# marcelodallaqua/TensorDiffEq

Measured on AMD Instinct MI355X. Metric: collocation-pts/sec + L2 rel-error, Allen-Cahn SA-PINN @ 1/2/4/8 GPU, higher is better.
Workload: dtype bf16; 1 GPU; model=Allen-Cahn SA-PINN tanh MLP [2,128,128,128,128,1], problem=ac-sa, global_batch=50000, parallelism=dp1, points_per_gpu=50000, backend=hip, bc_points=IC 512 (SA) + periodic 2x201 (u, u_x)

## Files before the change

tensordiffeq_amd/csrc/jet_bf3.hip:

```cpp
#include "jet_fused3.h"
#include "optim_common.h"

__device__ __forceinline__ void pack_frag(const float* __restrict__ P, bf16x8* __restrict__ img, const NetDims& d,
                                          int WT, int transposed, int e) {
  const int KB = WT / 2;
  {
    const int lane = e & 63, frag = e >> 6;
    const int kb = frag % KB, o = (frag / KB) % WT, layer = frag / (KB * WT) + 1;
    const int p = lane & 15, g = lane >> 4, row = 16 * o + p;
    const float* K = P + off_layer(d, layer);
    bf16x8 hi, lo;
#pragma unroll
    for (int j = 0; j < 8; ++j) {
      const int kf = 32 * kb + (j < 4 ? 4 * g + j : 16 + 4 * g + j - 4);
      const int in = transposed ? kf : row, out = transposed ? row : kf;
      const int win = hw(d, layer - 1), wout = hw(d, layer);
      const float v = (in < win && out < wout) ? K[in * wout + out] : 0.f;
      const __bf16 h = (__bf16)v;
      hi[j] = h;
      lo[j] = (__bf16)(v - (float)h);
    }
    img[(size_t)(frag * 2) * 64 + lane] = hi;
    img[(size_t)(frag * 2 + 1) * 64 + lane] = lo;
  }
}

__device__ __forceinline__ void pack_aux(const float* __restrict__ P, float* __restrict__ aux, const NetDims& d,
                                         int W, int e) {
  {
    float v = 0.f;
    const int w0 = hw(d, 0), wl = hw(d, d.n_hidden - 1);
    if (e < aux_b0(d, W)) {
      const int j = e / W, f = e - j * W;
      if (f < w0) v = P[j * w0 + f];
    } else if (e < aux_bh(d, W)) {
      const int f = e - aux_b0(d, W);
      if (f < w0) v = P[d.d_in * w0 + f];
    } else if (e < aux_ko(d, W)) {
      const int r = e - aux_bh(d, W), i = r / W + 1, f = r - (i - 1) * W;
      if (f < hw(d, i)) v = P[off_layer(d, i) + hw(d, i - 1) * hw(d, i) + f];
    } else if (e < aux_bo(d, W)) {
      const int r = e - aux_ko(d, W), f = r >> 2, q = r & 3;
      if (f < wl && q < d.d_out) v = P[off_layer(d, d.n_hidden) + f * d.d_out + q];
    } else {
      const int q = e - aux_bo(d, W);
      if (q < d.d_out) v = P[off_layer(d, d.n_hidden) + wl * d.d_out + q];
    }
    aux[e] = v;
  }
}

__global__ void __launch_bounds__(256) pack_all_kernel(const float* __restrict__ P, bf16x8* __restrict__ fimg,
                                                       bf16x8* __restrict__ bimg, float* __restrict__ aux, NetDims d,
                                                       int WT) {
  const int nf = (d.n_hidden - 1) * WT * (WT / 2) * 64;
  const int total = 2 * nf + aux_floats(d, 16 * WT);
  for (int e = blockIdx.x * 256 + threadIdx.x; e < total; e += gridDim.x * 256) {
    if (e < nf)
      pack_frag(P, fimg, d, WT, 1, e);
    else if (e < 2 * nf)
      pack_frag(P, bimg, d, WT, 0, e - nf);
    else
      pack_aux(P, aux, d, 16 * WT, e - 2 * nf);
  }
}

struct TailBook {
  const float* lpart;
  int n_lblocks, n_terms, n_scal;
  float* losses;
  float* total;
  float* dscal;
  float* hist;
  int64_t hist_rows;
  int64_t* epoch;
  float* best_loss;
  int64_t* best_epoch;
  int* improved;
  Counters cnt;
};

__global__ void __launch_bounds__(256) tail_reduce1_kernel(const float* __restrict__ slab, float* __restrict__ part,
                                                           int nwg, int Pst, int chunks, int nqb, int half, int c0,
                                                           TailBook tb) {
  if ((int)blockIdx.x < nqb) {
    const int q = blockIdx.x * 256 + threadIdx.x, c = c0 + (int)blockIdx.y;
    if (half) {
      if (8 * q < Pst) slab_reduce1_body8(slab, part, nwg, Pst, chunks, q, c);
    } else if (4 * q < Pst) {
      slab_reduce1_body<false>(slab, part, nwg, Pst, chunks, q, c);
    }
    return;
  }
  if (blockIdx.y != 0) return;
  __shared__ float sh[256];
  const int ns = tb.n_terms + tb.n_scal;
  for (int slot = 0; slot < ns; ++slot) {
    float s = 0.f;
    for (int b = threadIdx.x; b < tb.n_lblocks; b += 256) s += tb.lpart[(size_t)b * ns + slot];
    sh[threadIdx.x] = s;
    __syncthreads();
    for (int k = 128; k > 0; k >>= 1) {
      if ((int)threadIdx.x < k) sh[threadIdx.x] += sh[threadIdx.x + k];
      __syncthreads();
    }
    if (threadIdx.x == 0) {
      if (slot < tb.n_terms) tb.losses[slot] = sh[0];
      else tb.dscal[slot - tb.n_terms] = sh[0];
    }
    __syncthreads();
  }
  if (threadIdx.x == 0 && tb.hist == nullptr && tb.total != nullptr) {
    float s = 0.f;
    for (int t = 0; t < tb.n_terms; ++t) s += tb.losses[t];
    *tb.total = s;
  }
  if (threadIdx.x == 0 && tb.hist != nullptr)
    step_book_body(tb.total, tb.losses, tb.n_terms, 1, tb.hist, tb.hist_rows, tb.epoch, tb.best_loss, tb.best_epoch,
                   tb.improved, tb.cnt);
}

__global__ void __launch_bounds__(256) slab_reduce2_bf3(const float* __restrict__ part, float* __restrict__ grad, int P,
                                                        int Pst, int chunks, const float* __restrict__ gx) {
  const int q = blockIdx.x * 256 + threadIdx.x;
  if (4 * q >= P) return;
  const f32x4 a = slab_reduce2_sum(part, Pst, chunks, q);
#pragma unroll
  for (int e = 0; e < 4; ++e)
    if (4 * q + e < P) grad[4 * q + e] = gx != nullptr ? a[e] + gx[4 * q + e] : a[e];
}

__global__ void __launch_bounds__(256) tail_adam_kernel(AdamArgs args, const float* __restrict__ part, int Pst,
                                                        int chunks, const int* __restrict__ improved,
                                                        float* __restrict__ snap, TailImg ti,
                                                        const float* __restrict__ gx) {
  const bool do_snap = snap != nullptr && *improved != 0;
  const int64_t total = args.start[args.ngroups];
  for (int64_t idx = (int64_t)blockIdx.x * 256 + threadIdx.x; idx < total; idx += (int64_t)gridDim.x * 256) {
    const int gi = adam_group_of(args, idx);
    const AdamGroup gr = args.grp[gi];
    const int64_t e = idx - args.start[gi];
    const bool th = gi == 0;
    float g;
    if (th && part != nullptr) {
      float a0 = 0.f, a1 = 0.f;
      int c = 0;
      for (; c + 7 < chunks; c += 8) {
        float v[8];
#pragma unroll
        for (int k = 0; k < 8; ++k) v[k] = part[(size_t)(c + k) * Pst + e];
#pragma unroll
        for (int k = 0; k < 8; k += 2) {
          a0 += v[k];
          a1 += v[k + 1];
        }
      }
      for (; c + 1 < chunks; c += 2) {
        a0 += part[(size_t)c * Pst + e];
        a1 += part[(size_t)(c + 1) * Pst + e];
      }
      if (c < chunks) a0 += part[(size_t)c * Pst + e];
      g = a0 + a1;
      if (gx != nullptr) g += gx[e];
      const_cast<float*>(gr.g)[e] = g;
    } else {
      g = gr.g[e];
    }
    float p = gr.p[e], m = gr.m[e], v = gr.v[e];
    if (do_snap && th) snap[e] = p;
    adam_elem(p, gr.sign * g, m, v, gr.b1, gr.b2, gr.eps, adam_lr_t(gr));
    gr.p[e] = p;
    gr.m[e] = m;
    gr.v[e] = v;
    if (th && ti.fimg != nullptr) scatter_param(p, (int)e, ti);
  }
}

namespace {

int64_t img_floats(int WT, int n_hidden) {
  return (int64_t)(n_hidden > 1 ? n_hidden - 1 : 0) * WT * (WT / 2) * 128 * 4;
}

int64_t aux_alloc(int d_in, int n_hidden, int W) { return ((int64_t)(d_in + n_hidden + 4) * W + 4 + 3) / 4 * 4; }

int64_t stage_floats(int N, int WT, int S, int lo) {
  const int64_t nwg = (N + 63) / 64;
  return bf3_gstage(WT, S, lo != 0) ? nwg * 4 * stage_wave_elems(WT, S, true) * 2 : 0;
}

int bf3_rows(int N, const NetDims& d, int WT, int S, int lo) {
  const int pts_b = 16 * bwd_waves(WT, lo != 0, S);
  return (N + pts_b - 1) / pts_b;
}

int launch_pack(const float* P, bf16x8* fimg, bf16x8* bimg, float* aux, NetDims d, int WT, hipStream_t st) {
  const int total = 2 * (d.n_hidden - 1) * WT * (WT / 2) * 64 + aux_floats(d, 16 * WT);
  int blocks = (total + 255) / 256;
  if (blocks > 1024) blocks = 1024;
  hipLaunchKernelGGL(pack_all_kernel, dim3(blocks), dim3(256), 0, st, P, fimg, bimg, aux, d, WT);
  TDQ_CHECK_LAUNCH();
  return 0;
}

bool bf3_ok(int WT, int S, int d_in, int d_out, int n_hidden) {
  return (WT == 2 || WT == 4 || WT == 8 || (WT == 16 && S <= 4)) && S >= 1 && S <= TDQ_MAXS &&
         d_in <= TDQ_MAXD && d_out <= TDQ_MAXO && n_hidden >= 1;
}

int dispatch(bool fwd, int WT, int S, int nso, const Bf3Args& a) {
  switch (WT) {
    case 2: return fwd ? bf3_fwd_w2(S, nso, a) : bf3_bwd_w2(S, nso, a);
    case 4: return fwd ? bf3_fwd_w4(S, nso, a) : bf3_bwd_w4(S, nso, a);
    case 8: return fwd ? bf3_fwd_w8(S, nso, a) : bf3_bwd_w8(S, nso, a);
    case 16: return fwd ? bf3_fwd_w16(S, nso, a) : bf3_bwd_w16(S, nso, a);
    default: return (int)hipErrorInvalidValue;
  }
}

}

extern "C" {

int64_t tdq_jet_bf3_scratch_floats(int N, int d_in, const int* widths, int n_hidden, int S, int lo) {
  NetDims d;
  if (!make_dims(d, d_in, widths, 0, 1, n_hidden)) return -1;
  const int WT = width_tiles(d.width);
  if (WT < 2) return -1;
  const int64_t nwg = (N + 63) / 64;
  const int64_t hs = (int64_t)n_hidden * nwg * S * 4 * WT * 256;
  return hs + 2 * img_floats(WT, n_hidden) + aux_alloc(d_in, n_hidden, 16 * WT) + stage_floats(N, WT, S, lo);
}

int64_t tdq_jet_bf3_slab_floats(int N, int d_in, const int* widths, int d_out, int n_hidden) {
  NetDims d;
  if (!make_dims(d, d_in, widths, 0, d_out, n_hidden)) return -1;
  const int WT = width_tiles(d.width);
  if (WT < 2) return -1;
  int nwg = (N + 63) / 64;
  const int fz = (N + 15) / 16 < fz_cus() ? (N + 15) / 16 : fz_cus();
  if (fz > nwg) nwg = fz;
  const int64_t P = slab_stride(param_count(d));
  return ((int64_t)nwg + slab_chunks(nwg)) * P;
}

int64_t tdq_slab_floats_rows(int rows, int d_in, const int* widths, int d_out, int n_hidden) {
  NetDims d;
  if (rows < 1 || !make_dims(d, d_in, widths, 0, d_out, n_hidden)) return -1;
  return ((int64_t)rows + slab_chunks(rows)) * slab_stride(param_count(d));
}

static inline void scratch_images(float* scratch, int n_hidden, int WT, float** img, float** bimg, float** aux) {
  *img = scratch;
  *bimg = *img + img_floats(WT, n_hidden);
  *aux = *bimg + img_floats(WT, n_hidden);
}

static inline bf16x4* scratch_stage(float* scratch, int N, int d_in, int n_hidden, int S, int WT, int lo) {
  if (!bf3_gstage(WT, S, lo != 0)) return nullptr;
  float *img, *bimg, *aux;
  scratch_images(scratch, n_hidden, WT, &img, &bimg, &aux);
  return reinterpret_cast<bf16x4*>(aux + aux_alloc(d_in, n_hidden, 16 * WT));
}

static inline float* scratch_hs(float* scratch, int N, int d_in, int n_hidden, int S, int WT, int lo) {
  return scratch + 2 * img_floats(WT, n_hidden) + aux_alloc(d_in, n_hidden, 16 * WT) + stage_floats(N, WT, S, lo);
}

int tdq_jet_fwd_bf3_range(const float* X, const float* P, float* J, float* scratch, int N, int p_lo, int p_hi,
                          int d_in, const int* widths, int d_out, int n_hidden, int S, const int* spec, int lo, int pack,
                          void* stream) {
  if (N <= 0) return 0;
  if (p_lo < 0 || p_lo % 128 != 0 || p_hi > N || p_hi <= p_lo || (p_hi != N && p_hi % 128 != 0))
    return (int)hipErrorInvalidValue;
  NetDims d;
  if (!make_dims(d, d_in, widths, 0, d_out, n_hidden)) return (int)hipErrorInvalidValue;
  const int WT = width_tiles(d.width);
  JetSpec sp;
  if (!bf3_ok(WT, S, d_in, d_out, n_hidden)) return (int)hipErrorInvalidValue;
  const int nso = spec_nso(S, spec);
  if (nso < 0 || !make_spec(S, spec, sp)) return (int)hipErrorInvalidValue;
  hipStream_t st = reinterpret_cast<hipStream_t>(stream);
  float* Hs = scratch_hs(scratch, N, d_in, n_hidden, S, WT, lo);
  float *img, *bimg, *aux;
  scratch_images(scratch, n_hidden, WT, &img, &bimg, &aux);
  if (pack) {
    int rc = launch_pack(P, reinterpret_cast<bf16x8*>(img), reinterpret_cast<bf16x8*>(bimg), aux, d, WT, st);
    if (rc) return rc;
  }
  Bf3Args a{X, aux, reinterpret_cast<const bf16x8*>(img), nullptr, J, Hs, nullptr, N, 0, d, sp, st, lo,
            scratch_stage(scratch, N, d_in, n_hidden, S, WT, lo), p_lo, p_hi};
  return dispatch(true, WT, S, nso, a);
}

int tdq_jet_fwd_bf3_ex(const float* X, const float* P, float* J, float* scratch, int N, int d_in, const int* widths,
                       int d_out, int n_hidden, int S, const int* spec, int lo, int pack, void* stream) {
  return tdq_jet_fwd_bf3_range(X, P, J, scratch, N, 0, N, d_in, widths, d_out, n_hidden, S, spec, lo, pack, stream);
}

int tdq_jet_fwd_bf3(const float* X, const float* P, float* J, float* scratch, int N, int d_in, const int* widths,
                    int d_out, int n_hidden, int S, const int* spec, int lo, void* stream) {
  return tdq_jet_fwd_bf3_ex(X, P, J, scratch, N, d_in, widths, d_out, n_hidden, S, spec, lo, 1, stream);
}

int tdq_jet_bf3_pack(const float* P, float* scratch, int N, int d_in, const int* widths, int d_out, int n_hidden, int S,
                     void* stream) {
  NetDims d;
  if (!make_dims(d, d_in, widths, 0, d_out, n_hidden)) return (int)hipErrorInvalidValue;
  const int WT = width_tiles(d.width);
  if (!bf3_ok(WT, S, d_in, d_out, n_hidden)) return (int)hipErrorInvalidValue;
  float *img, *bimg, *aux;
  scratch_images(scratch, n_hidden, WT, &img, &bimg, &aux);
  return launch_pack(P, reinterpret_cast<bf16x8*>(img), reinterpret_cast<bf16x8*>(bimg), aux, d, WT,
                     reinterpret_cast<hipStream_t>(stream));
}

int tdq_jet_bwd_bf3_range(const float* X, const float* dJ, const float* Hs, float* work, int N, int p_lo, int p_hi,
                          int d_in, const int* widths, int d_out, int n_hidden, int S, const int* spec, int lo,
                          void* stream) {
  if (N <= 0) return 0;
  if (p_lo < 0 || p_lo % 128 != 0 || p_hi > N || p_hi <= p_lo || (p_hi != N && p_hi % 128 != 0))
    return (int)hipErrorInvalidValue;
  NetDims d;
  if (!make_dims(d, d_in, widths, 0, d_out, n_hidden)) return (int)hipErrorInvalidValue;
  const int WT = width_tiles(d.width);
  JetSpec sp;
  if (!bf3_ok(WT, S, d_in, d_out, n_hidden)) return (int)hipErrorInvalidValue;
  const int nso = spec_nso(S, spec);
  if (nso < 0 || !make_spec(S, spec, sp)) return (int)hipErrorInvalidValue;
  hipStream_t st = reinterpret_cast<hipStream_t>(stream);
  const int Ptot = param_count(d);
  float* scr = const_cast<float*>(Hs);
  float *img, *bimg, *aux;
  scratch_images(scr, n_hidden, WT, &img, &bimg, &aux);
  Bf3Args a{X, aux, reinterpret_cast<const bf16x8*>(bimg), dJ, nullptr, scratch_hs(scr, N, d_in, n_hidden, S, WT, lo),
            work, N, slab_stride(Ptot), d, sp, st, lo, scratch_stage(scr, N, d_in, n_hidden, S, WT, lo), p_lo, p_hi};
  return dispatch(false, WT, S, nso, a);
}

int tdq_jet_bwd_bf3_ex(const float* X, const float* P, const float* dJ, const float* Hs, float* work, float* grad,
                       int N, int d_in, const int* widths, int d_out, int n_hidden, int S, const int* spec, int lo, int reduce,
                       void* stream) {
  if (N <= 0) return 0;
  (void)P;
  int rc = tdq_jet_bwd_bf3_range(X, dJ, Hs, work, N, 0, N, d_in, widths, d_out, n_hidden, S, spec, lo, stream);
  if (rc || !reduce) return rc;
  NetDims d;
  make_dims(d, d_in, widths, 0, d_out, n_hidden);
  const int WT = width_tiles(d.width);
  const int nwg_b = bf3_rows(N, d, WT, S, lo);
  const int Ptot = param_count(d);
  return tdq_slab_reduce_h(work, grad, nwg_b, Ptot, slab_chunks(nwg_b), (int)slab_half(lo != 0), stream);
}

int tdq_jet_bwd_bf3(const float* X, const float* P, const float* dJ, const float* Hs, float* work, float* grad,
                    int N, int d_in, const int* widths, int d_out, int n_hidden, int S, const int* spec, int lo,
                    void* stream) {
  return tdq_jet_bwd_bf3_ex(X, P, dJ, Hs, work, grad, N, d_in, widths, d_out, n_hidden, S, spec, lo, 1, stream);
}

int tdq_step_tail_bf3(float* work, float* grad, float* scratch, int N, int d_in, const int* widths, int d_out, int n_hidden,
                      int S, int lo, const float* lpart, int n_lblocks, int n_terms, int n_scal, float* losses,
                      float* total, float* dscal, float* hist, int64_t hist_rows, int64_t* epoch, float* best_loss,
                      int64_t* best_epoch, int* improved, double* const* counters, int ncnt, const void* groups,
                      int ngroups, float* snap, int c_first, const float* gx, int rows, void* stream) {
  NetDims d;
  if (!make_dims(d, d_in, widths, 0, d_out, n_hidden)) return (int)hipErrorInvalidValue;
  const int WT = width_tiles(d.width);
  if (!bf3_ok(WT, S, d_in, d_out, n_hidden) || ncnt < 0 || ncnt > TDQ_MAX_COUNTERS || n_lblocks < 0 ||
      n_terms < 0 || n_scal < 0)
    return (int)hipErrorInvalidValue;
  AdamArgs args;
  if (!adam_args_fill(args, reinterpret_cast<const AdamGroup*>(groups), ngroups, true))
    return (int)hipErrorInvalidValue;
  const int Ptot = param_count(d);
  if (args.grp[0].n != Ptot) return (int)hipErrorInvalidValue;
  args.grp[0].g = grad;
  hipStream_t st = reinterpret_cast<hipStream_t>(stream);
  const int nwg_b = rows > 0 ? rows : bf3_rows(N, d, WT, S, lo);
  const int Pst = slab_stride(Ptot), chunks = slab_chunks(nwg_b);
  if (c_first < 0 || c_first >= chunks) return (int)hipErrorInvalidValue;
  float* part = work + (size_t)nwg_b * Pst;
  TailBook tb;
  tb.lpart = lpart;
  tb.n_lblocks = n_lblocks;
  tb.n_terms = n_terms;
  tb.n_scal = n_scal;
  tb.losses = losses;
  tb.total = total;
  tb.dscal = dscal;
  tb.hist = hist;
  tb.hist_rows = hist_rows;
  tb.epoch = epoch;
  tb.best_loss = best_loss;
  tb.best_epoch = best_epoch;
  tb.improved = improved;
  tb.cnt.n = ncnt;
  for (int i = 0; i < TDQ_MAX_COUNTERS; ++i) tb.cnt.c[i] = i < ncnt ? counters[i] : nullptr;
  const int half = (int)slab_half(lo != 0);
  const int nqb = (Pst / (half ? 8 : 4) + 255) / 256;
  hipLaunchKernelGGL(tail_reduce1_kernel, dim3(nqb + 1, chunks - c_first), dim3(256), 0, st, work, part, nwg_b, Pst,
                     chunks, nqb, half, c_first, tb);
  TDQ_CHECK_LAUNCH();
  TailImg ti{nullptr, nullptr, nullptr, d, WT};
  if (scratch != nullptr) {
    float *img, *bimg, *aux;
    scratch_images(scratch, n_hidden, WT, &img, &bimg, &aux);
    ti.fimg = reinterpret_cast<__bf16*>(img);
    ti.bimg = reinterpret_cast<__bf16*>(bimg);
    ti.aux = aux;
  }
  const int64_t tot = args.start[ngroups];
  int64_t blocks = (tot + 255) / 256;
  if (blocks > 2048) blocks = 2048;
  if (blocks < 1) blocks = 1;
  hipLaunchKernelGGL(tail_adam_kernel, dim3((unsigned)blocks), dim3(256), 0, st, args, part, Pst, chunks, improved,
                     snap, ti, gx);
  TDQ_CHECK_LAUNCH();
  return 0;
}

int tdq_dp_tail_a_bf3(float* work, float* grad, int N, int d_in, const int* widths, int d_out, int n_hidden, int S, int lo,
                      const float* lpart, int n_lblocks, int n_terms, int n_scal, float* losses, float* dscal,
                      float* total, int c_first, const float* gx, int rows, int half_ovr, void* stream) {
  NetDims d;
  if (!make_dims(d, d_in, widths, 0, d_out, n_hidden)) return (int)hipErrorInvalidValue;
  const int WT = width_tiles(d.width);
  if (!bf3_ok(WT, S, d_in, d_out, n_hidden) || N < 1 || n_lblocks < 0 || n_terms < 0 || n_scal < 0)
    return (int)hipErrorInvalidValue;
  hipStream_t st = reinterpret_cast<hipStream_t>(stream);
  const int Ptot = param_count(d);
  const int nwg_b = rows > 0 ? rows : bf3_rows(N, d, WT, S, lo);
  const int Pst = slab_stride(Ptot), chunks = slab_chunks(nwg_b);
  if (c_first < 0 || c_first >= chunks) return (int)hipErrorInvalidValue;
  float* part = work + (size_t)nwg_b * Pst;
  TailBook tb{};
  tb.lpart = lpart;
  tb.n_lblocks = n_lblocks;
  tb.n_terms = n_terms;
  tb.n_scal = n_scal;
  tb.losses = losses;
  tb.dscal = dscal;
  tb.total = total;
  const int half = half_ovr >= 0 ? (half_ovr != 0) : (int)slab_half(lo != 0);
  const int nqb = (Pst / (half ? 8 : 4) + 255) / 256, nq2 = (Pst / 4 + 255) / 256;
  hipLaunchKernelGGL(tail_reduce1_kernel, dim3(nqb + 1, chunks - c_first), dim3(256), 0, st, work, part, nwg_b, Pst,
                     chunks, nqb, half, c_first, tb);
  TDQ_CHECK_LAUNCH();
  hipLaunchKernelGGL(slab_reduce2_bf3, dim3(nq2), dim3(256), 0, st, part, grad, Ptot, Pst, chunks, gx);
  TDQ_CHECK_LAUNCH();
  return 0;
}

int tdq_bf3_slab_geometry(int N, int d_in, const int* widths, int d_out, int n_hidden, int S, int lo, int* out) {
  NetDims d;
  if (!make_dims(d, d_in, widths, 0, d_out, n_hidden)) return (int)hipErrorInvalidValue;
  const int WT = width_tiles(d.width);
  if (!bf3_ok(WT, S, d_in, d_out, n_hidden) || N < 1) return (int)hipErrorInvalidValue;
  const int pts_b = 16 * bwd_waves(WT, lo != 0, S), nwg_b = bf3_rows(N, d, WT, S, lo),
            chunks = slab_chunks(nwg_b);
  out[0] = pts_b;
  out[1] = nwg_b;
  out[2] = chunks;
  out[3] = 0;
  return 0;
}

int tdq_slab_prereduce_bf3(float* work, int N, int d_in, const int* widths, int d_out, int n_hidden, int S, int lo,
                           int c0, int c1, void* stream) {
  NetDims d;
  if (!make_dims(d, d_in, widths, 0, d_out, n_hidden)) return (int)hipErrorInvalidValue;
  const int WT = width_tiles(d.width);
  if (!bf3_ok(WT, S, d_in, d_out, n_hidden) || N < 1) return (int)hipErrorInvalidValue;
  const int Ptot = param_count(d);
  const int nwg_b = bf3_rows(N, d, WT, S, lo);
  const int Pst = slab_stride(Ptot), chunks = slab_chunks(nwg_b);
  if (c0 < 0 || c1 > chunks || c1 <= c0) return (int)hipErrorInvalidValue;
  float* part = work + (size_t)nwg_b * Pst;
  const int half = (int)slab_half(lo != 0);
  const int nqb = (Pst / (half ? 8 : 4) + 255) / 256;
  TailBook tb{};
  hipLaunchKernelGGL(tail_reduce1_kernel, dim3(nqb, c1 - c0), dim3(256), 0, reinterpret_cast<hipStream_t>(stream),
                     work, part, nwg_b, Pst, chunks, nqb, half, c0, tb);
  TDQ_CHECK_LAUNCH();
  return 0;
}

int tdq_dp_tail_b_bf3(float* scratch, int N, int d_in, const int* widths, int d_out, int n_hidden, int S,
                      const void* groups, int ngroups, const int* improved, float* snap, void* stream) {
  NetDims d;
  if (!make_dims(d, d_in, widths, 0, d_out, n_hidden)) return (int)hipErrorInvalidValue;
  const int WT = width_tiles(d.width);
  if (!bf3_ok(WT, S, d_in, d_out, n_hidden)) return (int)hipErrorInvalidValue;
  AdamArgs args;
  if (!adam_args_fill(args, reinterpret_cast<const AdamGroup*>(groups), ngroups, true))
    return (int)hipErrorInvalidValue;
  if (args.grp[0].n != param_count(d)) return (int)hipErrorInvalidValue;
  TailImg ti{nullptr, nullptr, nullptr, d, WT};
  if (scratch != nullptr) {
    float *img, *bimg, *aux;
    scratch_images(scratch, n_hidden, WT, &img, &bimg, &aux);
    ti.fimg = reinterpret_cast<__bf16*>(img);
    ti.bimg = reinterpret_cast<__bf16*>(bimg);
    ti.aux = aux;
  }
  const int64_t tot = args.start[ngroups];
  int64_t blocks = (tot + 255) / 256;
  if (blocks > 2048) blocks = 2048;
  if (blocks < 1) blocks = 1;
  hipLaunchKernelGGL(tail_adam_kernel, dim3((unsigned)blocks), dim3(256), 0, reinterpret_cast<hipStream_t>(stream),
                     args, nullptr, 0, 0, improved, snap, ti, nullptr);
  TDQ_CHECK_LAUNCH();
  return 0;
}

int tdq_fused_step_launch(void* func, const float* X, float* scratch, float* work, int N, int d_in, const int* widths,
                          int d_out, int n_hidden, int S, const int* spec, int G, const void* lptrs,
                          float* lpart, int prow, int nacc, int lo, void* stream) {
  if (func == nullptr || N <= 0 || G < 1 || prow < 0 || nacc < 1 || lo < 0 || lo > 1)
    return (int)hipErrorInvalidValue;
  NetDims d;
  if (!make_dims(d, d_in, widths, 0, d_out, n_hidden)) return (int)hipErrorInvalidValue;
  const int WT = width_tiles(d.width);
  if (!bf3_ok(WT, S, d_in, d_out, n_hidden) || tdq_jet_fused_lds(d_in, widths, d_out, n_hidden, S, lo) < 0)
    return (int)hipErrorInvalidValue;
  const int PT = lo ? FZ3_PT : FZ_PT;
  if (G > (N + PT - 1) / PT) return (int)hipErrorInvalidValue;
  JetSpec sp;
  if (spec_nso(S, spec) < 0 || !make_spec(S, spec, sp)) return (int)hipErrorInvalidValue;
  float *img, *bimg, *aux;
  scratch_images(scratch, n_hidden, WT, &img, &bimg, &aux);
  FzParams P{};
  P.X = X;
  P.aux = aux;
  P.fimg = reinterpret_cast<const bf16x8*>(img);
  P.bimg = reinterpret_cast<const bf16x8*>(bimg);
  P.slab = work;
  P.N = N;
  P.Pst = slab_stride(param_count(d));
  P.ntiles = (N + PT - 1) / PT;
  P.d = d;
  P.lptrs = reinterpret_cast<const FzLossPtrs*>(lptrs);
  P.lpart = lpart;
  P.prow = prow;
  P.nacc = nacc;
  void* args[] = {(void*)&P};
  return (int)hipModuleLaunchKernel((hipFunction_t)func, (unsigned)G, 1, 1, 64 * FZ_WAVES, 1, 1, 0,
                                    reinterpret_cast<hipStream_t>(stream), args, nullptr);
}

int tdq_fused_params_size() { return (int)sizeof(FzParams); }

int tdq_img_target(float* scratch, int d_in, const int* widths, int d_out, int n_hidden, void* out, int out_bytes) {
  NetDims d;
  if (scratch == nullptr || out == nullptr || !make_dims(d, d_in, widths, 0, d_out, n_hidden)) return -1;
  const int WT = width_tiles(d.width);
  if (WT < 2 || out_bytes < (int)sizeof(TailImg)) return -1;
  float *img, *bimg, *aux;
  scratch_images(scratch, n_hidden, WT, &img, &bimg, &aux);
  TailImg ti{reinterpret_cast<__bf16*>(img), reinterpret_cast<__bf16*>(bimg), aux, d, WT};
  *reinterpret_cast<TailImg*>(out) = ti;
  return (int)sizeof(TailImg);
}

}
```

tensordiffeq_amd/csrc/jet_common.h:

```cpp
#pragma once
#include "common.h"

#define TDQ_MAXS 8
#define TDQ_MAXD 8
#define TDQ_MAXO 4

struct JetSpec {
  int stype[TDQ_MAXS];
  int var[TDQ_MAXS];
  float selA[TDQ_MAXS][TDQ_MAXS];
  float selB[TDQ_MAXS][TDQ_MAXS];
  int ia[TDQ_MAXS], ib[TDQ_MAXS];
};

#define TDQ_MAXL 16

struct NetDims {
  int d_in, width, d_out, n_hidden;
  int lw[TDQ_MAXL];
  int lo[TDQ_MAXL + 1];
  int uniform;
};

__host__ __device__ __forceinline__ int off_layer(const NetDims& d, int i) { return d.lo[i]; }
__host__ __device__ __forceinline__ int hw(const NetDims& d, int i) { return d.lw[i]; }

static inline bool make_dims(NetDims& d, int d_in, const int* widths, int width, int d_out, int n_hidden) {
  if (n_hidden < 1 || n_hidden > TDQ_MAXL || d_in < 1 || d_out < 1) return false;
  d.d_in = d_in;
  d.d_out = d_out;
  d.n_hidden = n_hidden;
  int mx = 0, off = 0, prev = d_in;
  for (int i = 0; i < TDQ_MAXL; ++i) d.lw[i] = 0;
  for (int i = 0; i < n_hidden; ++i) {
    const int w = widths ? widths[i] : width;
    if (w < 1) return false;
    d.lw[i] = w;
    d.lo[i] = off;
    off += prev * w + w;
    prev = w;
    mx = w > mx ? w : mx;
  }
  d.lo[n_hidden] = off;
  for (int i = n_hidden + 1; i <= TDQ_MAXL; ++i) d.lo[i] = off;
  d.width = mx;
  d.uniform = 1;
  for (int i = 0; i < n_hidden; ++i) d.uniform &= d.lw[i] == mx;
  return true;
}

static inline int param_count(const NetDims& d) { return d.lo[d.n_hidden] + d.lw[d.n_hidden - 1] * d.d_out + d.d_out; }

__device__ __forceinline__ size_t zs_index(int layer, int nwg, int wg, int S, int s, int w, int WT,
                                           int t, int lane) {
  return ((((((size_t)layer * nwg + wg) * S + s) * 4 + w) * WT + t) * 256) + (unsigned)(lane * 4);
}

static inline int width_tiles(int width) {
  int wt = (width + 15) / 16;
  if (wt <= 1) return 1;
  if (wt <= 2) return 2;
  if (wt <= 4) return 4;
  if (wt <= 8) return 8;
  if (wt <= 16) return 16;
  return -1;
}

static inline int param_count(int d_in, int width, int d_out, int n_hidden) {
  return d_in * width + width + (n_hidden - 1) * (width * width + width) + width * d_out + d_out;
}

static inline NetDims uniform_dims(int d_in, int width, int d_out, int n_hidden) {
  NetDims d;
  make_dims(d, d_in, nullptr, width, d_out, n_hidden);
  return d;
}

static inline bool make_spec(int S, const int* spec, JetSpec& sp) {
  if (S < 1 || S > TDQ_MAXS) return false;
  for (int s = 0; s < TDQ_MAXS; ++s) {
    const int ty = s < S ? spec[3 * s] : 0, a = s < S ? spec[3 * s + 1] : 0, b = s < S ? spec[3 * s + 2] : 0;
    sp.stype[s] = ty;
    sp.var[s] = ty == 1 ? a : 0;
    sp.ia[s] = ty == 2 ? a : 0;
    sp.ib[s] = ty == 2 ? b : 0;
    for (int q = 0; q < TDQ_MAXS; ++q) {
      sp.selA[s][q] = (ty == 2 && q == a) ? 1.f : 0.f;
      sp.selB[s][q] = (ty == 2 && q == b) ? 1.f : 0.f;
    }
    if (ty == 2 && (a <= 0 || a >= S || b <= 0 || b >= S || spec[3 * a] != 1 || spec[3 * b] != 1)) return false;
    if (ty == 1 && a < 0) return false;
  }
  return true;
}

static inline int spec_nso(int S, const int* spec) {
  int nso = 0, prev = 0;
  for (int s = 0; s < S; ++s) {
    const int ty = spec[3 * s];
    if (ty < prev || (s == 0) != (ty == 0)) return -1;
    prev = ty;
    nso += ty == 2;
  }
  if (nso > 0 && S - 1 - nso < 1) return -1;
  return nso;
}

static inline int slab_stride(int P) { return (P + 7) & ~7; }

#ifndef TDQ_SLAB_CHUNKS
#define TDQ_SLAB_CHUNKS 8
#endif
static inline int slab_chunks(int nwg) {
  if (nwg < 2048) return nwg < TDQ_SLAB_CHUNKS ? nwg : TDQ_SLAB_CHUNKS;
  const int c = nwg / 256;
  return c < TDQ_SLAB_CHUNKS ? TDQ_SLAB_CHUNKS : (c > 256 ? 256 : c);
}
__host__ __device__ inline int slab_chunk_lo(int nwg, int chunks, int c) {
  return (int)(((long long)nwg * c) / chunks);
}

template <bool H>
__device__ __forceinline__ f32x4 slab_ld4(const void* __restrict__ slab, size_t row, int Pst, int q) {
  if constexpr (H) {
    const uint2 u = *reinterpret_cast<const uint2*>(reinterpret_cast<const unsigned short*>(slab) + row * Pst + 4 * q);
    return f32x4{__uint_as_float(u.x << 16), __uint_as_float(u.x & 0xffff0000u), __uint_as_float(u.y << 16),
                 __uint_as_float(u.y & 0xffff0000u)};
  } else {
    return reinterpret_cast<const f32x4*>(slab)[row * (size_t)(Pst >> 2) + q];
  }
}

template <bool H = false>
__device__ __forceinline__ void slab_reduce1_body(const void* __restrict__ slab, float* __restrict__ part, int nwg,
                                                  int Pst, int chunks, int q, int c) {
  const int lo = slab_chunk_lo(nwg, chunks, c), hi = slab_chunk_lo(nwg, chunks, c + 1);
  const size_t row = (size_t)(Pst >> 2);
  f32x4 a0 = zero4(), a1 = zero4(), a2 = zero4(), a3 = zero4();
  int wgi = lo;
  for (; wgi + 3 < hi; wgi += 4) {
    a0 += slab_ld4<H>(slab, wgi, Pst, q);
    a1 += slab_ld4<H>(slab, wgi + 1, Pst, q);
    a2 += slab_ld4<H>(slab, wgi + 2, Pst, q);
    a3 += slab_ld4<H>(slab, wgi + 3, Pst, q);
  }
  for (; wgi < hi; ++wgi) a0 += slab_ld4<H>(slab, wgi, Pst, q);
  reinterpret_cast<f32x4*>(part)[(size_t)c * row + q] = (a0 + a1) + (a2 + a3);
}

__device__ __forceinline__ void bf8_add(f32x4& lo, f32x4& hi, const uint4 u) {
  lo += f32x4{__uint_as_float(u.x << 16), __uint_as_float(u.x & 0xffff0000u), __uint_as_float(u.y << 16),
              __uint_as_float(u.y & 0xffff0000u)};
  hi += f32x4{__uint_as_float(u.z << 16), __uint_as_float(u.z & 0xffff0000u), __uint_as_float(u.w << 16),
              __uint_as_float(u.w & 0xffff0000u)};
}
__device__ __forceinline__ void slab_reduce1_body8(const void* __restrict__ slab, float* __restrict__ part, int nwg,
                                                   int Pst, int chunks, int q8, int c) {
  const int lo = slab_chunk_lo(nwg, chunks, c), hi = slab_chunk_lo(nwg, chunks, c + 1);
  const uint4* s8 = reinterpret_cast<const uint4*>(slab) + q8;
  const size_t rs = (size_t)(Pst >> 3);
  f32x4 a0 = zero4(), a1 = zero4(), a2 = zero4(), a3 = zero4();
  f32x4 b0 = zero4(), b1 = zero4(), b2 = zero4(), b3 = zero4();
  int w = lo;
  for (; w + 7 < hi; w += 8) {
    uint4 u[8];
#pragma unroll
    for (int k = 0; k < 8; ++k) u[k] = s8[(size_t)(w + k) * rs];
    bf8_add(a0, b0, u[0]);
    bf8_add(a1, b1, u[1]);
    bf8_add(a2, b2, u[2]);
    bf8_add(a3, b3, u[3]);
    bf8_add(a0, b0, u[4]);
    bf8_add(a1, b1, u[5]);
    bf8_add(a2, b2, u[6]);
    bf8_add(a3, b3, u[7]);
  }
  for (; w + 3 < hi; w += 4) {
    const uint4 u0 = s8[(size_t)w * rs], u1 = s8[(size_t)(w + 1) * rs], u2 = s8[(size_t)(w + 2) * rs],
                u3 = s8[(size_t)(w + 3) * rs];
    bf8_add(a0, b0, u0);
    bf8_add(a1, b1, u1);
    bf8_add(a2, b2, u2);
    bf8_add(a3, b3, u3);
  }
  for (; w < hi; ++w) bf8_add(a0, b0, s8[(size_t)w * rs]);
  f32x4* p4 = reinterpret_cast<f32x4*>(part) + (size_t)c * (size_t)(Pst >> 2) + 2 * q8;
  p4[0] = (a0 + a1) + (a2 + a3);
  p4[1] = (b0 + b1) + (b2 + b3);
}

__device__ __forceinline__ f32x4 slab_reduce2_sum(const float* __restrict__ part, int Pst, int chunks, int q) {
  const f32x4* p4 = reinterpret_cast<const f32x4*>(part) + q;
  const size_t row = (size_t)(Pst >> 2);
  f32x4 a0 = zero4(), a1 = zero4();
  int c = 0;
  for (; c + 7 < chunks; c += 8) {
    f32x4 v[8];
#pragma unroll
    for (int k = 0; k < 8; ++k) v[k] = p4[(size_t)(c + k) * row];
#pragma unroll
    for (int k = 0; k < 8; k += 2) {
      a0 += v[k];
      a1 += v[k + 1];
    }
  }
  for (; c + 1 < chunks; c += 2) {
    a0 += p4[(size_t)c * row];
    a1 += p4[(size_t)(c + 1) * row];
  }
  if (c < chunks) a0 += p4[(size_t)c * row];
  return a0 + a1;
}

extern "C" int tdq_slab_reduce(float* work, float* grad, int nwg, int P, int chunks, void* stream);
extern "C" int tdq_slab_reduce_h(float* work, float* grad, int nwg, int P, int chunks, int half, void* stream);
```

tensordiffeq_amd/csrc/jet_fused.h:

```cpp
#pragma once
#include "jet_bf3.h"

#ifndef FZ_TS_TILE
#define FZ_TS_TILE 0
#endif
#define FZ_TS(k) \
  do {                \
    if (t == t0 + FZ_TS_TILE) TDQ_TS(k); \
  } while (0)

#define FZ_PT 32
#define FZ_WAVES 8

__host__ __device__ constexpr int fz_nslot(int LM) { return LM < 2 ? 2 : LM; }
__host__ __device__ constexpr int fz_img_elems(int WT, int S, int LM) {
  return (S + 1) * fz_nslot(LM) * FZ_PT * bf3_img_rs(WT);
}
struct FzFl {
  int bh, ko, bo, xs, ubs, part, pq, outp, lpre, total;
};
__host__ __device__ constexpr FzFl fz_fl(int W, int d_in, int S, int LM, int PT, int NQ, int NW, int DO = 1) {
  FzFl f{};
  f.bh = (d_in + 1) * W;
  f.ko = (d_in + LM + 1) * W;
  f.bo = (d_in + LM + 5) * W;
  f.xs = (f.bo + 4 + 3) / 4 * 4;
  f.ubs = f.xs + PT * TDQ_MAXD;
  f.part = f.ubs + S * PT * 4;
  f.pq = (LM + 1) * W + d_in * W + 4 * W;
  f.outp = f.part + NQ * f.pq + 4;
  f.lpre = f.outp + NW * S * PT * DO;
  f.total = f.lpre + PT;
  return f;
}
__host__ __device__ inline int fz_lds_bytes(const NetDims& d, int WT, int S, int LM) {
  return fz_img_elems(WT, S, LM) * 2 + fz_fl(16 * WT, d.d_in, S, LM, FZ_PT, 2, 4, d.d_out).total * 4;
}

template <int WT, int S, int NSO, bool CHEAP, int DIN>
__device__ __forceinline__ void fz_h0(const JetSpec& sp, const float* aux, const float* xrow, int t, int g,
                                      f32x4 (&h)[S]) {
  constexpr int S1 = S - 1 - NSO, SO = 1 + S1, W = 16 * WT;
  static_assert(DIN > 0, "fz_h0: compile-time input width");
  const int f0 = 16 * t + 4 * g;
  f32x4 z = *reinterpret_cast<const f32x4*>(aux + DIN * W + f0);
  {
    float x[DIN];
#pragma unroll
    for (int j = 0; j < DIN; ++j) x[j] = xrow[j];
#pragma unroll
    for (int c = 0; c < 4; ++c) {
      float a = z[c];
#pragma unroll
      for (int j = 0; j < DIN; ++j) a = fmaf(x[j], aux[j * W + f0 + c], a);
      z[c] = a;
    }
  }
  f32x4 ka[S];
  ka[0] = zero4();
#pragma unroll
  for (int s = 1; s < SO; ++s) ka[s] = *reinterpret_cast<const f32x4*>(aux + sp.var[s] * W + f0);
#pragma unroll
  for (int s = SO; s < S; ++s) ka[s] = zero4();
  f32x4 kp[S];
#pragma unroll
  for (int s = SO; s < S; ++s) kp[s] = sel_first<S, S1>(ka, sp.ia[s], sp.selA[s]) * sel_first<S, S1>(ka, sp.ib[s], sp.selB[s]);
#pragma unroll
  for (int c = 0; c < 4; ++c) {
    float hv, s1;
    if constexpr (CHEAP) {
      const float e = __builtin_amdgcn_exp2f(fminf(z[c], 15.f) * 2.8853900817779268f);
      const float r = __builtin_amdgcn_rcpf(1.f + e);
      hv = fmaf(-2.f, r, 1.f);
      s1 = (4.f * e) * (r * r);
    } else {
      tanh_s1(z[c], hv, s1);
    }
    const float s2 = -2.f * hv * s1;
    h[0][c] = hv;
#pragma unroll
    for (int s = 1; s < SO; ++s) h[s][c] = s1 * ka[s][c];
#pragma unroll
    for (int s = SO; s < S; ++s) h[s][c] = s2 * kp[s][c];
  }
}

struct FzLane {
  int lo, r2;
};
template <int RS>
__device__ __forceinline__ FzLane fz_lane(int p, int g) {
  const int ch = g ^ ((p >> 2) & 3), rsw = (p & 8) << 3;
  return FzLane{p * RS + 4 * ch + rsw, 2 * rsw};
}
template <int RS>
__device__ __forceinline__ int fz_at(const FzLane& L, int q, int t) {
  return L.lo - ((t >> 2) & 1) * L.r2 + 16 * q * RS + 16 * t;
}
template <int RS>
__device__ __forceinline__ void fz_put(__bf16* im, const FzLane& L, int q, int t, bf16x4 v) {
  *reinterpret_cast<bf16x4*>(im + fz_at<RS>(L, q, t)) = v;
}
template <int RS>
__device__ __forceinline__ bf16x4 fz_get(const __bf16* im, const FzLane& L, int q, int t) {
  return *reinterpret_cast<const bf16x4*>(im + fz_at<RS>(L, q, t));
}
template <int RS>
__device__ __forceinline__ bf16x8 fz_bfrag(const __bf16* im, const FzLane& L, int q, int kb) {
  return cat8(fz_get<RS>(im, L, q, 2 * kb), fz_get<RS>(im, L, q, 2 * kb + 1));
}
__device__ __forceinline__ f32x4 fz_bf4(bf16x4 v) {
  const u32x2 u = __builtin_bit_cast(u32x2, v);
  return f32x4{__uint_as_float(u[0] << 16), __uint_as_float(u[0] & 0xffff0000u), __uint_as_float(u[1] << 16),
               __uint_as_float(u[1] & 0xffff0000u)};
}
template <int WT, int S>
__device__ __forceinline__ void fz_get_h(const __bf16* im, const FzLane& L, int q, int t, f32x4 (&h)[S]) {
  constexpr int RS = bf3_img_rs(WT), SIMG = FZ_PT * RS;
  h[0] = fz_bf4(fz_get<RS>(im, L, q, t)) + fz_bf4(fz_get<RS>(im + S * SIMG, L, q, t));
#pragma unroll
  for (int s = 1; s < S; ++s) h[s] = fz_bf4(fz_get<RS>(im + s * SIMG, L, q, t));
}

template <int WT, int OPW>
struct FzW {
  bf16x8 a[WT / 2][OPW];
};
constexpr int FZ_WAHEAD = 2;
template <int WT, int OPW>
__device__ __forceinline__ void fz_load_w(FzW<WT, OPW>& w, const bf16x8* __restrict__ wimg, int layer, int o0, int l,
                                          int kb) {
  constexpr int KB = WT / 2, NSTEP = WT * KB;
  if (kb >= KB) return;
  const Tl Wi = tl_make(wimg + (size_t)(layer - 1) * NSTEP * 128, l);
#pragma unroll
  for (int oo = 0; oo < OPW; ++oo) {
    bf16x8 unused;
    img_frag<false>(Wi, (o0 + oo) * KB + kb, w.a[kb][oo], unused);
  }
}
template <int WT, int OPW>
__device__ __forceinline__ void fz_pre_w(FzW<WT, OPW>& w, const bf16x8* __restrict__ wimg, int layer, int o0, int l) {
#pragma unroll
  for (int kb = 0; kb < FZ_WAHEAD; ++kb) fz_load_w<WT, OPW>(w, wimg, layer, o0, l, kb);
}

template <int WT, int S, int OPW>
__device__ __forceinline__ void fz_gemm(f32x4 (&acc)[OPW][S], FzW<WT, OPW>& w, const bf16x8* __restrict__ wimg, int layer,
                                        int o0, int l, const __bf16* im, int q, const FzLane& L) {
  constexpr int KB = WT / 2, RS = bf3_img_rs(WT), SIMG = FZ_PT * RS;
#pragma unroll
  for (int oo = 0; oo < OPW; ++oo)
#pragma unroll
    for (int s = 0; s < S; ++s) acc[oo][s] = zero4();
#pragma unroll
  for (int kb = 0; kb < KB; ++kb) {
    fz_load_w<WT, OPW>(w, wimg, layer, o0, l, kb + FZ_WAHEAD);
    bf16x8 b[S];
#pragma unroll
    for (int s = 0; s < S; ++s) b[s] = fz_bfrag<RS>(im + s * SIMG, L, q, kb);
#pragma unroll
    for (int oo = 0; oo < OPW; ++oo)
#pragma unroll
      for (int s = 0; s < S; ++s) acc[oo][s] = mfma_bf(w.a[kb][oo], b[s], acc[oo][s]);
    __builtin_amdgcn_sched_barrier(0);
  }
}

struct FzTr {
  int a1, a2, z1, z2;
};
template <int RS, int NR, int NC>
__device__ __forceinline__ FzTr fz_tr(int r0, int c0, int l) {
  const int g = l >> 4;
  const int tr_row = 8 * g + ((l & 15) >> 2);
  const int swz = (g & 1) << 6;
  const int tr_col1 = 4 * ((l & 3) ^ ((2 * g) & 3)), tr_col2 = 4 * ((l & 3) ^ ((2 * g + 1) & 3));
  static_assert((NR == 4 || NR <= 2) && (NC == 4 || NC <= 2), "fz_tr: tile blocks of 1, 2 or 4");
  return FzTr{tr_row * RS + tr_col1 + ((16 * r0) ^ swz), (tr_row + 4) * RS + tr_col2 + ((16 * r0) ^ swz),
              tr_row * RS + tr_col1 + ((16 * c0) ^ swz), (tr_row + 4) * RS + tr_col2 + ((16 * c0) ^ swz)};
}
template <int WT, int S, int NR, int NC, bool SB = true, int SIMG = FZ_PT * bf3_img_rs(WT)>
__device__ __forceinline__ void fz_dk(f32x4 (&dk)[NR][NC], const __bf16* H, const __bf16* Z, int r0, int c0, int l) {
  const auto [a1, a2, z1, z2] = fz_tr<bf3_img_rs(WT), NR, NC>(r0, c0, l);
#pragma unroll
  for (int s = 0; s < S; ++s) {
    bf16x8 A[NR], B[NC];
#pragma unroll
    for (int r = 0; r < NR; ++r) A[r] = cat8(tr_read(H + s * SIMG + a1 + 16 * r), tr_read(H + s * SIMG + a2 + 16 * r));
#pragma unroll
    for (int c = 0; c < NC; ++c) B[c] = cat8(tr_read(Z + s * SIMG + z1 + 16 * c), tr_read(Z + s * SIMG + z2 + 16 * c));
#pragma unroll
    for (int r = 0; r < NR; ++r)
#pragma unroll
      for (int c = 0; c < NC; ++c) dk[r][c] = mfma_bf(A[r], B[c], dk[r][c]);
    if constexpr (SB) __builtin_amdgcn_sched_barrier(0);
  }
}

struct FzLossPtrs {
  const float* val[16];
  const float* lam[8];
  float* dlam[8];
  const float* scal[8];
};

struct FzParams {
  const float* X;
  const float* aux;
  const bf16x8* fimg;
  const bf16x8* bimg;
  float* slab;
  int N, Pst, ntiles;
  NetDims d;
  const FzLossPtrs* lptrs;
  float* lpart;
  int prow, nacc;
};

template <int S, int PT, int NW>
__device__ __forceinline__ float fz_jsum(const float* jv, int s, int k, float bo) {
  float a = jv[s * PT + k];
#pragma unroll
  for (int w = 1; w < NW; ++w) a += jv[(w * S + s) * PT + k];
  return s == 0 ? a + bo : a;
}
template <int S, int PT, int NW, int DOUT>
__device__ __forceinline__ float fz_jsum_q(const float* jv, int s, int k, int q, const float* bo) {
  static_assert(DOUT >= 2 && DOUT <= 4, "fz_jsum_q: 2-4 outputs");
  float a = 0.f;
#pragma unroll
  for (int w = 0; w < NW; ++w) {
    const float* e = jv + ((w * S + s) * PT + k) * DOUT;
    float v;
    if constexpr (DOUT == 2) v = (*reinterpret_cast<const f32x2*>(e))[q];
    else if constexpr (DOUT == 4) v = (*reinterpret_cast<const f32x4*>(e))[q];
    else v = e[q];
    a = w == 0 ? v : a + v;
  }
  if constexpr (NW > 1) return s == 0 ? a + bo[q] : a;
  return a;
}


template <int PT>
__device__ __forceinline__ void fz_stage(float* xs, float* lpre, int tid, float v) {
  if (tid < PT * TDQ_MAXD) xs[tid] = v;
  else if (tid < PT * TDQ_MAXD + PT) lpre[tid - PT * TDQ_MAXD] = v;
}

template <int WT, int LM, int NAUX>
__device__ __forceinline__ void fz_setup(const FzParams& P, float* aux, int tid) {
  const float* __restrict__ aux_g = P.aux;
  const int G = gridDim.x, gi = blockIdx.x;
  bf16x8 wpf[2];
  {
    constexpr int NI16 = LM * WT * (WT / 2) * 128 * 4 * 4 / 16;
    const int xw = gi >> 3, nx = (G + 7) >> 3;
#pragma unroll
    for (int k = 0; k < 2; ++k) {
      const int e = (xw + k * nx) * 64 * FZ_WAVES + tid;
      wpf[k] = e < 2 * NI16 ? (e < NI16 ? P.fimg[e] : P.bimg[e - NI16]) : bf16x8{};
    }
  }
  for (int e = tid; e < NAUX; e += 64 * FZ_WAVES) aux[e] = e < aux_floats(P.d, 16 * WT) ? aux_g[e] : 0.f;
  asm volatile("" ::"v"(wpf[0]), "v"(wpf[1]));
}

template <int WT, int S, int NSO, int LM, class LossF>
__device__ __forceinline__ void fz_body(const FzParams& P, char* lds_raw) {
  const int N = P.N, Pst = P.Pst, ntiles = P.ntiles;
  const NetDims& d = P.d;
  constexpr JetSpec sp = LossF::SPEC;
  constexpr int DIN = LossF::DIN, DOUT = LossF::DOUT;
  constexpr int W = 16 * WT, OPW = WT / 4, RS = bf3_img_rs(WT), SIMG = FZ_PT * RS, PT = FZ_PT;
  constexpr int NR = WT / 4, NC = WT / 2;
  constexpr int ZS = 0;
  static_assert(OPW >= 1 && OPW * 4 == WT, "fused step: WT = 4 or 8");
  static_assert(LM >= 2, "fused step keeps h_LM in h_0's slot");
  __bf16* img = reinterpret_cast<__bf16*>(lds_raw);
  auto slot = [&](int k) { return img + k * (S + 1) * SIMG; };
  constexpr FzFl F = fz_fl(W, DIN, S, LM, PT, 2, 4, DOUT);
  float* aux = reinterpret_cast<float*>(img + fz_img_elems(WT, S, LM));
  float *xs = aux + F.xs, *ubs = aux + F.ubs, *part = aux + F.part, *outp = aux + F.outp, *lpre = aux + F.lpre;

  const int tid = threadIdx.x, l = tid & 63, p = l & 15, g = l >> 4;
  const int w = __builtin_amdgcn_readfirstlane(tid >> 6);
  const int q = w >> 2, wo = w & 3;
  const int G = gridDim.x, gi = blockIdx.x;
  const int t0 = (int)((long long)ntiles * gi / G), t1 = (int)((long long)ntiles * (gi + 1) / G);
  const int r0 = NR * (w >> 1), c0 = NC * (w & 1);
  const int o0 = wo * OPW;
  const int row = 16 * q + p;
  const FzLane L = fz_lane<RS>(p, g);
  float* accB = part + q * F.pq;
  float* accK0 = accB + (LM + 1) * W;
  float* accKo = accK0 + DIN * W;
  const bf16x8* Wimg = P.fimg;
  const bf16x8* Kimg = P.bimg;

  static_assert(FZ_PT * TDQ_MAXD + FZ_PT <= 64 * FZ_WAVES, "one element per thread");
  const float* __restrict__ X = P.X;
  float xpre = 0.f;
  auto fetch = [&](int tt) {
    const int pb = tt * FZ_PT;
    if (tid < FZ_PT * TDQ_MAXD) {
      const int pt = tid / TDQ_MAXD, j = tid - pt * TDQ_MAXD;
      const int n = min(pb + pt, N - 1);
      xpre = j < DIN ? X[(size_t)n * DIN + j] : 0.f;
    } else if (tid < FZ_PT * TDQ_MAXD + FZ_PT) {
      xpre = LossF::pre(pb + tid - FZ_PT * TDQ_MAXD, N, *P.lptrs);
    }
  };
  if (t0 < t1) fetch(t0);
  fz_setup<WT, LM, F.xs>(P, aux, tid);
  f32x4 dk[LM][NR][NC];
  float lacc[LossF::NACC];
  float bo_q[DOUT];
#pragma unroll
  for (int qo = 0; qo < DOUT; ++qo) bo_q[qo] = 0.f;
#pragma unroll
  for (int k = 0; k < LossF::NACC; ++k) lacc[k] = 0.f;
#pragma unroll
  for (int i = 0; i < LM; ++i)
#pragma unroll
    for (int r = 0; r < NR; ++r)
#pragma unroll
      for (int c = 0; c < NC; ++c) dk[i][r][c] = zero4();
  for (int e = tid; e < 2 * F.pq + 4; e += 64 * FZ_WAVES) part[e] = 0.f;
  const float* Ko = aux + F.ko;

  auto layer0 = [&](int oo, f32x4(&h)[S]) { fz_h0<WT, S, NSO, true, DIN>(sp, aux, xs + row * TDQ_MAXD, o0 + oo, g, h); };

  int t = t0;
  FzW<WT, OPW> wf;
  TDQ_TS(0);
  while (t < t1) {
    const int pb = t * PT;
    asm volatile("" : "+s"(Wimg), "+s"(Kimg));
    __syncthreads();
    fz_stage<PT>(xs, lpre, tid, xpre);
    if (t + 1 < t1) fetch(t + 1);
    __syncthreads();
    FZ_TS(1);

#pragma unroll
    for (int oo = 0; oo < OPW; ++oo) {
      f32x4 h[S];
      layer0(oo, h);
#pragma unroll
      for (int s = 0; s < S; ++s) fz_put<RS>(slot(0) + s * SIMG, L, q, o0 + oo, cvt_hi4(h[s]));
    }
    fz_pre_w<WT, OPW>(wf, Wimg, 1, o0, l);
    __syncthreads();
    FZ_TS(2);

#pragma unroll
    for (int ly = 1; ly <= LM; ++ly) {
      const float* bi = aux + F.bh + (ly - 1) * W;
      f32x4 acc[OPW][S];
      fz_gemm<WT, S, OPW>(acc, wf, Wimg, ly, o0, l, slot(ly - 1), q, L);
      FZ_TS(1 + 2 * ly);
      f32x4 hq[OPW][S];
#pragma unroll
      for (int oo = 0; oo < OPW; ++oo) {
        const int to = o0 + oo;
        f32x4 z[S], h[S];
#pragma unroll
        for (int s = 0; s < S; ++s) z[s] = acc[oo][s];
        z[0] += *reinterpret_cast<const f32x4*>(bi + 16 * to + 4 * g);
        tanh_jet_f<S, NSO>(sp, z, h);
        __bf16* im = slot(ly < LM ? ly : ZS);
        bf16x4 hi, lo;
        split4(h[0], hi, lo);
        fz_put<RS>(im, L, q, to, hi);
        fz_put<RS>(im + S * SIMG, L, q, to, lo);
#pragma unroll
        for (int s = 1; s < S; ++s) fz_put<RS>(im + s * SIMG, L, q, to, cvt_hi4(h[s]));
        if (ly == LM) {
#pragma unroll
          for (int s = 0; s < S; ++s) hq[oo][s] = h[s];
        }
      }
      if (ly == LM) {
#pragma unroll
        for (int s = 0; s < S; ++s) {
          float a[DOUT];
#pragma unroll
          for (int qo = 0; qo < DOUT; ++qo) a[qo] = 0.f;
#pragma unroll
          for (int oo = 0; oo < OPW; ++oo)
#pragma unroll
            for (int c = 0; c < 4; ++c)
#pragma unroll
              for (int qo = 0; qo < DOUT; ++qo)
                a[qo] = fmaf(hq[oo][s][c], Ko[(16 * (o0 + oo) + 4 * g + c) * 4 + qo], a[qo]);
#pragma unroll
          for (int qo = 0; qo < DOUT; ++qo) {
            const float r = col4_sum(a[qo]);
            if (g == 0) outp[((wo * S + s) * FZ_PT + row) * DOUT + qo] = r;
          }
        }
      }
      if (ly < LM) fz_pre_w<WT, OPW>(wf, Wimg, ly + 1, o0, l);
      __syncthreads();
      FZ_TS(2 + 2 * ly);
    }

    int tl = tid;
    asm volatile("" : "+v"(tl));
    if constexpr (DOUT == 1) {
      if (tl < PT) LossF::template eval<S, PT, 4>(outp, xs, tl, pb + tl, N, *P.lptrs, ubs, lacc, lpre[tl], aux[F.bo]);
    } else {
      if (tl < PT) LossF::template eval<S, PT, 4>(outp, xs, tl, pb + tl, N, *P.lptrs, ubs, lacc, lpre[tl], aux + F.bo);
    }
    __syncthreads();
    FZ_TS(9);
    tl = tid;
    asm volatile("" : "+v"(tl));
    if (tl < PT) {
#pragma unroll
      for (int qo = 0; qo < DOUT; ++qo) bo_q[qo] += ubs[tl * 4 + qo];
    }
#pragma unroll
    for (int oo = 0; oo < OPW; ++oo) {
      const int to = o0 + oo;
      __bf16* im = slot(ZS);
      f32x4 h[S], hb[S], zb[S];
      fz_get_h<WT, S>(im, L, q, to, h);
      f32x4 kq[DOUT], pp[DOUT];
#pragma unroll
      for (int qo = 0; qo < DOUT; ++qo) {
        pp[qo] = zero4();
#pragma unroll
        for (int c = 0; c < 4; ++c) kq[qo][c] = Ko[(16 * to + 4 * g + c) * 4 + qo];
      }
#pragma unroll
      for (int s = 0; s < S; ++s) {
#pragma unroll
        for (int qo = 0; qo < DOUT; ++qo) {
          const float ub = ubs[(s * FZ_PT + row) * 4 + qo];
          hb[s] = qo == 0 ? kq[0] * ub : hb[s] + kq[qo] * ub;
          pp[qo] += h[s] * ub;
        }
      }
#pragma unroll
      for (int qo = 0; qo < DOUT; ++qo) {
        const float r = row16_sum4(pp[qo]);
        if ((p & 3) == 0) accKo[(16 * to + 4 * g + (p >> 2)) * 4 + qo] += r;
      }
      tanh_jet_b<S, NSO>(sp, h, hb, zb);
      const float r = row16_sum4(zb[0]);
      if ((p & 3) == 0) accB[LM * W + 16 * to + 4 * g + (p >> 2)] += r;
#pragma unroll
      for (int s = 0; s < S; ++s) fz_put<RS>(im + s * SIMG, L, q, to, cvt_hi4(zb[s]));
    }
    fz_pre_w<WT, OPW>(wf, Kimg, LM, o0, l);
    __syncthreads();
#pragma unroll
    for (int ly = LM; ly >= 1; --ly) {
      const __bf16* Z = slot(ly == LM ? ZS : ly);
      __bf16* H = slot(ly - 1);
      const int tb = 10 + 5 * (LM - ly);
      f32x4 acc[OPW][S];
      fz_gemm<WT, S, OPW>(acc, wf, Kimg, ly, o0, l, Z, q, L);
      FZ_TS(tb);
      bf16x4 zbh[OPW][S];
      float rb[OPW];
      if (ly >= 2) {
#pragma unroll
        for (int oo = 0; oo < OPW; ++oo) {
          const int to = o0 + oo;
          f32x4 h[S], zb[S];
          fz_get_h<WT, S>(H, L, q, to, h);
          tanh_jet_b<S, NSO>(sp, h, acc[oo], zb);
          rb[oo] = row16_sum4(zb[0]);
#pragma unroll
          for (int s = 0; s < S; ++s) zbh[oo][s] = cvt_hi4(zb[s]);
        }
      }
      fz_dk<WT, S, NR, NC, false>(dk[ly - 1], H, Z, r0, c0, l);
      FZ_TS(tb + 1);
      if (ly >= 2) {
        __syncthreads();
        FZ_TS(tb + 2);
#pragma unroll
        for (int oo = 0; oo < OPW; ++oo) {
          const int to = o0 + oo;
          if ((p & 3) == 0) accB[(ly - 1) * W + 16 * to + 4 * g + (p >> 2)] += rb[oo];
#pragma unroll
          for (int s = 0; s < S; ++s) fz_put<RS>(H + s * SIMG, L, q, to, zbh[oo][s]);
        }
      } else {
#pragma unroll
        for (int oo = 0; oo < OPW; ++oo) {
          const int to = o0 + oo;
          f32x4 h[S], zb[S];
          fz_get_h<WT, S>(H, L, q, to, h);
          tanh_jet_b<S, NSO>(sp, h, acc[oo], zb);
          const int fo = 16 * to + 4 * g + (p >> 2);
          {
            const float r = row16_sum4(zb[0]);
            if ((p & 3) == 0) accB[fo] += r;
          }
#pragma unroll
          for (int j = 0; j < DIN; ++j) {
            const float xj = xs[row * TDQ_MAXD + j];
            f32x4 vv;
#pragma unroll
            for (int c = 0; c < 4; ++c) {
              float a = xj * zb[0][c];
              constexpr int SO = S - NSO;
#pragma unroll
              for (int s = 1; s < SO; ++s) a += (sp.var[s] == j) ? zb[s][c] : 0.f;
              vv[c] = a;
            }
            const float r = row16_sum4(vv);
            if ((p & 3) == 0) accK0[j * W + fo] += r;
          }
        }
      }
      FZ_TS(tb + 3);
      if (ly == 2) {
        if (LM == 2) __syncthreads();
#pragma unroll
        for (int oo = 0; oo < OPW; ++oo) {
          f32x4 h[S];
          layer0(oo, h);
          bf16x4 hi, lo;
          split4(h[0], hi, lo);
          fz_put<RS>(slot(0), L, q, o0 + oo, hi);
          fz_put<RS>(slot(0) + S * SIMG, L, q, o0 + oo, lo);
#pragma unroll
          for (int s = 1; s < S; ++s) fz_put<RS>(slot(0) + s * SIMG, L, q, o0 + oo, cvt_hi4(h[s]));
        }
      }
      if (ly >= 2) {
        fz_pre_w<WT, OPW>(wf, Kimg, ly - 1, o0, l);
        __syncthreads();
      }
      FZ_TS(tb + 4);
    }
    ++t;
  }
  TDQ_TS(62);

  __bf16* gs = reinterpret_cast<__bf16*>(P.slab) + (size_t)gi * Pst;
#pragma unroll
  for (int ly = 1; ly <= LM; ++ly) {
    const int voff = ((16 * r0 + 4 * g) * W + 16 * c0 + p) * 2;
    const Tl Gt = tl_make(gs + off_layer(d, ly), 0);
#pragma unroll
    for (int r = 0; r < NR; ++r)
#pragma unroll
      for (int c = 0; c < NC; ++c)
#pragma unroll
        for (int e = 0; e < 4; ++e)
          __builtin_amdgcn_raw_buffer_store_b16(__builtin_bit_cast(unsigned short, (__bf16)dk[ly - 1][r][c][e]),
                                                Gt.r, voff, ((16 * r + e) * W + 16 * c) * 2, 0);
  }
  __syncthreads();
  const float* pA = part;
  const float* pB = part + F.pq;
  for (int f = tid; f < W; f += 64 * FZ_WAVES) {
    gs[DIN * W + f] = (__bf16)(pA[f] + pB[f]);
    for (int ly = 1; ly <= LM; ++ly)
      gs[off_layer(d, ly) + W * W + f] = (__bf16)(pA[ly * W + f] + pB[ly * W + f]);
    for (int j = 0; j < DIN; ++j) {
      const int k = (LM + 1) * W + j * W + f;
      gs[j * W + f] = (__bf16)(pA[k] + pB[k]);
    }
#pragma unroll
    for (int qo = 0; qo < DOUT; ++qo) {
      const int k = (LM + 1 + DIN) * W + f * 4 + qo;
      gs[off_layer(d, LM + 1) + f * DOUT + qo] = (__bf16)(pA[k] + pB[k]);
    }
  }
  if (w == 0) {
#pragma unroll
    for (int qo = 0; qo < DOUT; ++qo) {
      const float bq = col4_sum(row16_sum(bo_q[qo]));
      if (l == 0) gs[off_layer(d, LM + 1) + W * DOUT + qo] = (__bf16)bq;
    }
#pragma unroll
    for (int k = 0; k < LossF::NACC; ++k) {
      const float v = col4_sum(row16_sum(lacc[k]));
      if (l == 0 && k < P.nacc) P.lpart[(size_t)(P.prow + gi) * P.nacc + k] = v;
    }
  }
  TDQ_TS(63);
}

#ifndef __HIPCC_RTC__
int fz_cus();
extern "C" int tdq_jet_fused_lds(int d_in, const int* widths, int d_out, int n_hidden, int S, int lo);
#endif
```

tensordiffeq_amd/csrc/optim.hip:

```cpp
#include "optim_common.h"

__global__ void __launch_bounds__(256) adam_multi_kernel(AdamArgs args, const int* __restrict__ improved,
                                                          float* __restrict__ snap) {
  const bool do_snap = snap != nullptr && *improved != 0;
  const int64_t total = args.start[args.ngroups];
  for (int64_t slot = (int64_t)blockIdx.x * 256 + threadIdx.x; slot < total;
       slot += (int64_t)gridDim.x * 256) {
    const int gi = adam_group_of(args, slot);
    const AdamGroup gr = args.grp[gi];
    const int64_t e0 = (slot - args.start[gi]) * 4;
    const float sg = gr.sign, b1 = gr.b1, b2 = gr.b2, eps = gr.eps;
    const float lr_t = adam_lr_t(gr);
    const bool aligned = ((((uintptr_t)gr.p) | ((uintptr_t)gr.g) | ((uintptr_t)gr.m) | ((uintptr_t)gr.v)) & 15) == 0;
    if (aligned && e0 + 4 <= gr.n) {
      f32x4 p = *reinterpret_cast<const f32x4*>(gr.p + e0);
      if (do_snap && gi == 0) *reinterpret_cast<f32x4*>(snap + e0) = p;
      const f32x4 g = *reinterpret_cast<const f32x4*>(gr.g + e0);
      f32x4 m = *reinterpret_cast<const f32x4*>(gr.m + e0);
      f32x4 v = *reinterpret_cast<const f32x4*>(gr.v + e0);
#pragma unroll
      for (int c = 0; c < 4; ++c) {
        float pc = p[c], mc = m[c], vc = v[c];
        adam_elem(pc, sg * g[c], mc, vc, b1, b2, eps, lr_t);
        p[c] = pc; m[c] = mc; v[c] = vc;
      }
      *reinterpret_cast<f32x4*>(gr.p + e0) = p;
      *reinterpret_cast<f32x4*>(gr.m + e0) = m;
      *reinterpret_cast<f32x4*>(gr.v + e0) = v;
    } else {
      for (int c = 0; c < 4; ++c) {
        const int64_t e = e0 + c;
        if (e < gr.n) {
          if (do_snap && gi == 0) snap[e] = gr.p[e];
          adam_elem(gr.p[e], sg * gr.g[e], gr.m[e], gr.v[e], b1, b2, eps, lr_t);
        }
      }
    }
  }
}

__global__ void __launch_bounds__(256) best_copy_kernel(const float* __restrict__ loss,
                                                         const float* __restrict__ best_loss,
                                                         const float* __restrict__ flat,
                                                         float* __restrict__ best_flat, int64_t n) {
  const float lv = *loss;
  if (!(lv < *best_loss)) return;
  for (int64_t i = (int64_t)blockIdx.x * 256 + threadIdx.x; i < n; i += (int64_t)gridDim.x * 256)
    best_flat[i] = flat[i];
}

__global__ void best_scalar_kernel(const float* __restrict__ loss, float* __restrict__ best_loss,
                                   int64_t* __restrict__ best_epoch, const int64_t* __restrict__ epoch) {
  const float lv = *loss;
  if (lv < *best_loss) {
    *best_loss = lv;
    *best_epoch = *epoch;
  }
}

__global__ void step_book_kernel(float* __restrict__ loss, const float* __restrict__ terms, int n_terms, int sum_terms,
                                 float* __restrict__ hist, int64_t hist_rows, int64_t* __restrict__ epoch,
                                 float* __restrict__ best_loss, int64_t* __restrict__ best_epoch,
                                 int* __restrict__ improved, Counters cnt) {
  step_book_body(loss, terms, n_terms, sum_terms, hist, hist_rows, epoch, best_loss, best_epoch, improved, cnt);
}

extern "C" {

int tdq_abi_version() { return 27; }

int tdq_step_book(float* loss, const float* terms, int n_terms, int sum_terms, float* hist, int64_t hist_rows,
                  int64_t* epoch, float* best_loss, int64_t* best_epoch, int* improved, double* const* counters,
                  int ncnt, void* stream) {
  if (ncnt < 0 || ncnt > TDQ_MAX_COUNTERS) return (int)hipErrorInvalidValue;
  Counters c;
  c.n = ncnt;
  for (int i = 0; i < TDQ_MAX_COUNTERS; ++i) c.c[i] = i < ncnt ? counters[i] : nullptr;
  hipLaunchKernelGGL(step_book_kernel, dim3(1), dim3(1), 0, reinterpret_cast<hipStream_t>(stream), loss, terms,
                     n_terms, sum_terms, hist, hist_rows, epoch, best_loss, best_epoch, improved, c);
  TDQ_CHECK_LAUNCH();
  return 0;
}

int tdq_adam_multi(const void* groups, int ngroups, const int* improved, float* snap, void* stream) {
  AdamArgs args;
  if (!adam_args_fill(args, reinterpret_cast<const AdamGroup*>(groups), ngroups)) return (int)hipErrorInvalidValue;
  const int64_t total = args.start[ngroups];
  if (total == 0) return 0;
  int64_t blocks = (total + 255) / 256;
  if (blocks > 2048) blocks = 2048;
  hipLaunchKernelGGL(adam_multi_kernel, dim3((unsigned)blocks), dim3(256), 0,
                     reinterpret_cast<hipStream_t>(stream), args, improved, snap);
  TDQ_CHECK_LAUNCH();
  return 0;
}

int tdq_best_track(const float* loss, float* best_loss, const float* flat, float* best_flat,
                   int64_t* best_epoch, const int64_t* epoch, int64_t n, void* stream) {
  hipStream_t st = reinterpret_cast<hipStream_t>(stream);
  int64_t blocks = (n + 255) / 256;
  if (blocks > 1024) blocks = 1024;
  if (blocks < 1) blocks = 1;
  hipLaunchKernelGGL(best_copy_kernel, dim3((unsigned)blocks), dim3(256), 0, st, loss, best_loss, flat,
                     best_flat, n);
  TDQ_CHECK_LAUNCH();
  hipLaunchKernelGGL(best_scalar_kernel, dim3(1), dim3(1), 0, st, loss, best_loss, best_epoch, epoch);
  TDQ_CHECK_LAUNCH();
  return 0;
}

}
```

tensordiffeq_amd/csrc/optim_common.h:

```cpp
#pragma once
#include "common.h"

#define TDQ_MAX_GROUPS 16
#define TDQ_MAX_COUNTERS 8

struct AdamGroup {
  float* p;
  const float* g;
  float* m;
  float* v;
  int64_t n;
  float sign;
  float lr, b1, b2, eps;
  float pad;
  const double* t;
};

struct AdamArgs {
  AdamGroup grp[TDQ_MAX_GROUPS];
  int64_t start[TDQ_MAX_GROUPS + 1];
  int ngroups;
};

struct Counters {
  double* c[TDQ_MAX_COUNTERS];
  int n;
};

__device__ __forceinline__ void adam_elem(float& p, float g, float& m, float& v, float b1, float b2,
                                          float eps, float lr_t) {
  m = fmaf(1.f - b1, g, b1 * m);
  v = fmaf(1.f - b2, g * g, b2 * v);
  p = p - lr_t * m / (sqrtf(v) + eps);
}

__device__ __forceinline__ float adam_lr_t(const AdamGroup& gr) {
  const double t = *gr.t;
  return (float)((double)gr.lr * sqrt(1.0 - pow((double)gr.b2, t)) / (1.0 - pow((double)gr.b1, t)));
}

__device__ __forceinline__ int adam_group_of(const AdamArgs& args, int64_t slot) {
  int gi = 0;
#pragma unroll
  for (int q = 1; q < TDQ_MAX_GROUPS; ++q)
    if (q < args.ngroups && slot >= args.start[q]) gi = q;
  return gi;
}

static inline bool adam_args_fill(AdamArgs& args, const AdamGroup* src, int ngroups, bool per_elem = false) {
  if (ngroups <= 0 || ngroups > TDQ_MAX_GROUPS) return false;
  args.ngroups = ngroups;
  args.start[0] = 0;
  for (int i = 0; i < TDQ_MAX_GROUPS; ++i) {
    if (i < ngroups) {
      args.grp[i] = src[i];
      args.start[i + 1] = args.start[i] + (per_elem ? src[i].n : (src[i].n + 3) / 4);
    } else {
      args.grp[i] = AdamGroup{nullptr, nullptr, nullptr, nullptr, 0, 1.f, 0.f, 0.f, 0.f, 0.f, 0.f, nullptr};
      args.start[i + 1] = args.start[i];
    }
  }
  return true;
}

__device__ __forceinline__ void step_book_body(float* __restrict__ loss, const float* __restrict__ terms,
                                               int n_terms, int sum_terms, float* __restrict__ hist,
                                               int64_t hist_rows, int64_t* __restrict__ epoch,
                                               float* __restrict__ best_loss, int64_t* __restrict__ best_epoch,
                                               int* __restrict__ improved, const Counters& cnt) {
  float lv = *loss;
  if (sum_terms) {
    lv = 0.f;
    for (int t = 0; t < n_terms; ++t) lv += terms[t];
    *loss = lv;
  }
  const int64_t ep = *epoch;
  if (ep >= 0 && ep < hist_rows) {
    float* row = hist + ep * (1 + n_terms);
    row[0] = lv;
    for (int t = 0; t < n_terms; ++t) row[1 + t] = terms[t];
  }
  const int imp = lv < *best_loss;
  if (imp) {
    *best_loss = lv;
    *best_epoch = ep;
  }
  *improved = imp;
  for (int i = 0; i < cnt.n; ++i) *cnt.c[i] += 1.0;
  *epoch = ep + 1;
}
```

tensordiffeq_amd/fit.py:

```python
from __future__ import annotations

import math
import os
import time

import torch

from .graphs import capture_graph
from .optimizers import adam as adam_mod
from .ops import fused


def _use_graphs(device):
    return (torch.device(device).type == "cuda" and os.environ.get("TDQ_NO_GRAPH", "0") != "1")


class _Bucket:

    def __init__(self, tensors, n_scalars):
        self.sizes = [t.numel() for t in tensors]
        self.n_scalars = n_scalars

    def pack(self, grads, scalars):
        return torch.cat([g.reshape(-1) for g in grads] + [s.reshape(1).to(grads[0].dtype) for s in scalars])

    def unpack(self, buf):
        out, off = [], 0
        for n in self.sizes:
            out.append(buf[off:off + n])
            off += n
        return out, buf[off:off + self.n_scalars]


def _term_list(terms):
    return list(terms.unbind()) if torch.is_tensor(terms) else list(terms)


class ParamGroup:

    def __init__(self, tensors, get_opt, sign=1.0, reduce=None):
        self.tensors = list(tensors)
        self.get_opt = get_opt
        self.sign = float(sign)
        self.reduce = list(reduce) if reduce is not None else [True] * len(self.tensors)


def default_bind(n_lambdas):
    def bind(alias):
        return {"params": alias[0], "lambdas": alias[1:1 + n_lambdas]}
    return bind


class AdamEngine:

    def __init__(self, solver, program, groups, n_steps_hint=0, lambdas=None, bind=None):
        self.s = solver
        self.program = program
        self.groups = [g for g in groups if g.tensors]
        self.flat = groups[0].tensors[0]
        self.lambdas = lambdas if lambdas is not None else []
        self.dist = solver.dist_ctx
        dev = self.flat.device
        self.device = dev
        self.state = solver._train_state(dev)
        self.term_names = [t.name for t in program.terms]
        self.graph_a = self.graph_b = None
        self.static_loss = None
        self.wrt = [t for g in self.groups for t in g.tensors]
        self.bind = bind if bind is not None else default_bind(len(self.lambdas))
        self.red_idx = [i for i, r in enumerate(r for g in self.groups for r in g.reduce) if r]
        self.points = PointPass(program, self.flat)
        self._fsrc = self._grad = self._dp_buf = self._sig = self.graph_k = self._graph_saved = None
        self._sum_terms = False
        self._bind_opts()
        self._ensure_hist(n_steps_hint)

    def _bind_opts(self):
        self.opts = [g.get_opt() for g in self.groups]
        self._tail_ok = None
        self.counters = [o.step_counter(self.device) for o in self.opts]
        self.moments = [[o.state_for(t) for t in g.tensors] for o, g in zip(self.opts, self.groups)]

    def _ensure_hist(self, n):
        st = self.state
        if "improved" not in st:
            st["improved"] = torch.zeros((), dtype=torch.int32, device=self.device)
        need = int(st["epoch_host"]) + int(n) + 1
        if st["hist"] is None or st["hist"].shape[0] < need:
            old = 0 if st["hist"] is None else st["hist"].shape[0]
            new = torch.full((max(need, 2 * old, 16), 1 + len(self.term_names)), float("nan"),
                             device=self.device)
            if st["hist"] is not None:
                new[: st["hist"].shape[0]] = st["hist"]
            st["hist"] = new
            self.graph_a = self.graph_b = None
            self.graph_k = None

    def _fused_map(self, fop):
        fl = fop.fl
        n_lam = len(self.lambdas)
        src = [("flat", 0)]
        for i in range(1, len(self.wrt)):
            if i <= n_lam:
                k = i - 1
                if k in fl.lam_slots:
                    src.append(("dlam", fl.lam_slots.index(k)))
                elif ("lam", k) in fl.scal_slots:
                    src.append(("dscal", fl.scal_slots.index(("lam", k))))
                else:
                    src.append(("zero", 0))
            else:
                k = i - 1 - n_lam
                src.append(("dscal", fl.scal_slots.index(("extra", k))) if ("extra", k) in fl.scal_slots
                           else ("zero", 0))
        return src

    def _fused_grads(self, fop, gflat, dlam, dscal):
        if self._fsrc is None:
            self._fsrc = self._fused_map(fop)
        grads = []
        for (kind, k), w in zip(self._fsrc, self.wrt):
            if kind == "flat":
                grads.append(gflat)
            elif kind == "dlam":
                g = dlam[k]
                rng = fop.fl.lam_offsets.get(fop.fl.lam_slots[k])
                if rng is not None:
                    full = torch.zeros(w.numel(), device=w.device)
                    full[rng[0]:rng[1]] = g
                    g = full
                grads.append(g.view_as(w))
            elif kind == "dscal":
                grads.append(dscal[k].view_as(w))
            else:
                grads.append(torch.zeros_like(w))
        return grads

    def _phase_a_fused(self, fop, for_step=False):
        from .ops import jet_hip
        prog = self.program
        hi = prog.hi_op
        J, saved = jet_hip.forward_raw(prog.X_all, self.flat, prog.net, prog.plan, prog.precision,
                                       rows=fop.fl.n_streams)
        if hi is not None:
            hi.forward(J, self.flat)
        total, losses, dJ, dlam, dscal = fop(J, with_total=not for_step)
        gflat = jet_hip.backward_raw(saved, dJ)
        if hi is not None:
            gflat = gflat + hi.backward(dJ, self.flat)
        grads = self._fused_grads(fop, gflat, dlam, dscal)
        return total, grads, losses

    def _phase_a(self, for_step=False):
        fop = getattr(self.program, "fused_op", None)
        self._sum_terms = fop is not None and for_step
        if fop is not None:
            return self._phase_a_fused(fop, for_step)
        alias = [t.detach().requires_grad_(True) for t in self.wrt]
        loss, vals = self.program.evaluate(**self.bind(alias))
        grads = torch.autograd.grad(loss, alias, allow_unused=True)
        grads = [torch.zeros_like(w) if g is None else g for g, w in zip(grads, alias)]
        terms = [vals[n].detach().reshape(()) for n in self.term_names]
        return loss.detach(), grads, terms

    def _reduce(self, loss, grads, terms):
        if not self.dist.is_distributed:
            return loss, grads, terms
        red_idx = self.red_idx
        red = [grads[i] for i in red_idx]
        terms = _term_list(terms)
        bucket = _Bucket(red, 1 + len(terms))
        buf = bucket.pack(red, [loss] + terms)
        self.dist.all_reduce_(buf)
        red_out, scal = bucket.unpack(buf)
        grads = list(grads)
        for i, g in zip(red_idx, red_out):
            grads[i] = g.view_as(grads[i])
        return scal[0], grads, scal[1:]

    def _book(self, loss, terms):
        st = self.state
        if "improved" not in st:
            st["improved"] = torch.zeros((), dtype=torch.int32, device=self.device)
        tv = terms if torch.is_tensor(terms) else (
            torch.stack([t.float().reshape(()) for t in terms]) if len(terms)
            else torch.zeros(0, device=self.device))
        fused.step_book(loss, tv.reshape(-1).float().contiguous(), st, self.counters,
                        sum_terms=self._sum_terms)

    def _opt_groups(self, grads):
        off = 0
        opt_groups = []
        for grp, opt, t, mom in zip(self.groups, self.opts, self.counters, self.moments):
            n = len(grp.tensors)
            items = [(p, g, m, v, grp.sign) for p, g, (m, v) in zip(grp.tensors, grads[off:off + n], mom)]
            opt_groups.append((items, t, opt.learning_rate, opt.beta_1, opt.beta_2, opt.epsilon))
            off += n
        return opt_groups

    def _phase_b(self, loss, grads, terms):
        st = self.state
        self._book(loss, terms)
        opt_groups = self._opt_groups(grads)
        snap = (st["best_flat"], st["improved"]) if self.groups[0].tensors[0] is self.flat else None
        fused.adam_multi_opts(opt_groups, snapshot=snap)
        return loss

    def _tail_eligible(self):
        if self._tail_ok is None:
            ok = self.points.eligible and self.groups[0].tensors[0] is self.flat
            if ok:
                probe = [(w, w, m, v, 1.0) for w, (m, v) in zip(self.wrt, (mv for ms in self.moments for mv in ms))]
                ok = fused.group_array([(probe, self.counters[0], 0.0, 0.0, 0.0, 0.0)]) is not None
            self._tail_ok = ok
        return self._tail_ok

    def _tail_step(self, in_graph):
        from .ops import jet_hip
        prog = self.program
        fop = prog.fused_op
        st = self.state
        if "improved" not in st:
            st["improved"] = torch.zeros((), dtype=torch.int32, device=self.device)
        if st["best_flat"].numel() != self.flat.numel():
            raise ValueError(f"best-weights snapshot has {st['best_flat'].numel()} elements, parameters "
                             f"{self.flat.numel()}")
        saved, work, pre, kw = self.points.run(pack=not in_graph)
        if self._grad is None:
            self._grad = torch.empty_like(self.flat)
        grad = self._grad
        grads = self._fused_grads(fop, grad, fop.dlam, fop.dscal)
        packed = fused.group_array(self._opt_groups(grads))
        if packed is None:
            raise RuntimeError("fused step tail: parameter groups do not fit one launch "
                               "(set TDQ_FUSED_TAIL=0)")
        hi = prog.hi_op
        jet_hip.step_tail(saved, work, grad, fop, st, self.counters, packed[0], packed[1], st["best_flat"],
                          write_images=in_graph, c_first=pre, gextra=hi.grad if hi is not None else None, **kw)
        self._tail_saved = saved
        return fop.total

    def _dp_tail_phase_b(self, loss, grads, terms):
        from .ops import jet_hip
        st = self.state
        self._book(loss, terms)
        if st["best_flat"].numel() != self.flat.numel():
            raise ValueError(f"best-weights snapshot has {st['best_flat'].numel()} elements, parameters "
                             f"{self.flat.numel()}")
        packed = fused.group_array(self._opt_groups(grads))
        if packed is None:
            raise RuntimeError("fused step tail: parameter groups do not fit one launch "
                               "(set TDQ_FUSED_TAIL=0)")
        jet_hip.dp_tail_b(self._tail_saved, packed[0], packed[1], st["improved"], st["best_flat"])
        return loss

    def _eager_step(self):
        if self._tail_eligible():
            if not self.dist.is_distributed:
                return self._tail_step(in_graph=False)
            self._dp_half_a_inplace(pack=True)
            self.dist.all_reduce_(self._bucket_buf)
            self._dp_half_b(True)
            return self.static_loss
        loss, grads, terms = self._phase_a(for_step=True)
        loss, grads, terms = self._reduce(loss, grads, terms)
        return self._phase_b(loss, grads, terms)

    def _capture(self):
        if self._tail_eligible():
            self.points.fused_step()
        stream = torch.cuda.Stream(device=self.device)
        stream.wait_stream(torch.cuda.current_stream(self.device))
        split = self.dist.is_distributed
        with torch.cuda.stream(stream):
            warm = self._eager_step()
            self.state["epoch_host"] += 1
        torch.cuda.current_stream(self.device).wait_stream(stream)
        torch.cuda.synchronize(self.device)
        pool = torch.cuda.graph_pool_handle()
        self._graph_saved = None
        if not split:
            tail = self._tail_eligible()
            g = torch.cuda.CUDAGraph()
            with capture_graph(g, pool=pool):
                self.static_loss = self._tail_step(in_graph=True) if tail else self._eager_step()
            self.graph_a, self.graph_b = g, None
            if tail:
                self._graph_saved = self._tail_saved
        else:
            tail = self._tail_eligible()
            self.dist.settle_collective(self._bucket_floats())
            if self._coll_in_graph():
                g = torch.cuda.CUDAGraph()
                with capture_graph(g, pool=pool):
                    self._dp_half_a(tail)
                    self.dist.all_reduce_(self._bucket_buf)
                    self._dp_half_b(tail)
                self.graph_a, self.graph_b = g, None
            else:
                ga = torch.cuda.CUDAGraph()
                with capture_graph(ga, pool=pool):
                    self._dp_half_a(tail)
                gb = torch.cuda.CUDAGraph()
                with capture_graph(gb, pool=pool):
                    self._dp_half_b(tail)
                self.graph_a, self.graph_b = ga, gb
            if tail:
                self._graph_saved = self._tail_saved
        return warm

    def _dp_half_a(self, tail):
        if tail:
            return self._dp_half_a_inplace()
        loss, grads, terms = self._phase_a(for_step=True)
        red_idx = self.red_idx
        red = [grads[i] for i in red_idx]
        terms = _term_list(terms)
        self._bucket = _Bucket(red, 1 + len(terms))
        self._bucket_buf = self._bucket.pack(red, [loss] + terms)
        self._grads_static = grads
        self._red_idx = red_idx

    def _dp_half_a_inplace(self, pack=False):
        from .ops import jet_hip
        prog = self.program
        fop = prog.fused_op
        saved, work, pre, kw = self.points.run(pack=pack)
        n_p = self.flat.numel()
        red_idx = self.red_idx
        if not red_idx or red_idx[0] != 0:
            raise RuntimeError("DP bucket: theta must be the first reduced tensor")
        others = [i for i in red_idx[1:]]
        sizes = [self.wrt[i].numel() for i in others]
        n_e, n_t = sum(sizes), fop.n_terms
        buf = self._dp_buf
        if buf is None or buf.numel() != n_p + n_e + 1 + n_t:
            buf = self._dp_buf = torch.empty(n_p + n_e + 1 + n_t, dtype=torch.float32, device=self.device)
        grad_view = buf[:n_p]
        hi = prog.hi_op
        jet_hip.dp_tail_a(saved, work, grad_view, fop, total=buf[n_p + n_e:n_p + n_e + 1],
                          losses=buf[n_p + n_e + 1:], c_first=pre, gextra=hi.grad if hi is not None else None, **kw)
        grads = self._fused_grads(fop, grad_view, fop.dlam, fop.dscal)
        if others:
            torch.cat([grads[i].reshape(-1) for i in others], out=buf[n_p:n_p + n_e])
        self._sum_terms = True
        self._tail_saved = saved
        self._bucket = _Bucket([grads[i] for i in red_idx], 1 + n_t)
        self._bucket_buf = buf
        self._grads_static = grads
        self._red_idx = red_idx

    def _dp_half_b(self, tail):
        red_out, scal = self._bucket.unpack(self._bucket_buf)
        grads = list(self._grads_static)
        for i, gg in zip(self._red_idx, red_out):
            grads[i] = gg.view_as(grads[i])
        self.static_loss = (self._dp_tail_phase_b if tail else self._phase_b)(scal[0], grads, scal[1:])

    def _capture_k(self, k):
        pool = torch.cuda.graph_pool_handle()
        g = torch.cuda.CUDAGraph()
        with capture_graph(g, pool=pool):
            for _ in range(k):
                if self.dist.is_distributed:
                    self._dp_half_a(True)
                    self.dist.all_reduce_(self._bucket_buf)
                    self._dp_half_b(True)
                    loss = self.static_loss
                else:
                    loss = self._tail_step(in_graph=True)
        self.graph_k, self.static_loss_k, self._k = g, loss, k

    def _bucket_floats(self):
        return sum(self.wrt[i].numel() for i in self.red_idx) + 1 + len(self.term_names)

    def _coll_in_graph(self):
        return self.dist.capturable(self._bucket_floats())

    def _replay(self):
        self.graph_a.replay()
        if self.graph_b is not None:
            self.dist.all_reduce_(self._bucket_buf)
            self.graph_b.replay()
        return self.static_loss

    def run(self, n_steps, progress=None, log_every=100, use_graph=None):
        if n_steps <= 0:
            return None
        opts = [g.get_opt() for g in self.groups]
        sig = [(o.learning_rate, o.beta_1, o.beta_2, o.epsilon) for o in opts]
        if any(a is not b for a, b in zip(opts, self.opts)) or self._sig not in (None, sig):
            self._bind_opts()
            self.graph_a = self.graph_b = None
            self.graph_k = None
        self._sig = sig
        self._ensure_hist(n_steps)
        use_graph = _use_graphs(self.device) if use_graph is None else use_graph
        st = self.state
        loss = None
        done = 0
        if use_graph and self.graph_a is None:
            loss = self._capture()
            done = 1
            if progress is not None and n_steps == 1:
                progress(1, float(loss))
        if use_graph and self.graph_a is not None and self._graph_saved is not None \
                and done < n_steps:
            from .ops import jet_hip
            jet_hip.pack_images(self._graph_saved)
        checked = int(st["epoch_host"]) - done
        K = self._unroll()
        if use_graph and self.graph_a is not None and K > 1 and n_steps - done >= K \
                and self.graph_k is None:
            self._capture_k(K)
        while done < n_steps:
            next_log = (done // log_every + 1) * log_every if progress is not None else n_steps
            if use_graph and K > 1 and self.graph_k is not None and n_steps - done >= K \
                    and done + K <= next_log:
                self.graph_k.replay()
                loss = self.static_loss_k
                done += K
                st["epoch_host"] += K
            else:
                loss = self._replay() if (use_graph and self.graph_a is not None) else self._eager_step()
                done += 1
                st["epoch_host"] += 1
            if progress is not None and (done % log_every == 0 or done == n_steps):
                checked = self._check_finite(checked)
                progress(done, float(loss))
        self._check_finite(checked)
        return loss

    def _unroll(self):
        if not self._tail_eligible() or (self.dist.is_distributed and not self._coll_in_graph()):
            return 1
        return max(1, int(os.environ.get("TDQ_STEP_UNROLL", "8")))

    def _check_finite(self, lo):
        st = self.state
        hi = int(st["epoch_host"])
        self.dist.check_health()
        if hi <= lo or os.environ.get("TDQ_NAN_CHECK", "1") == "0":
            return hi
        col = st["hist"][lo:hi, 0]
        if math.isfinite(float(col.sum())):
            return hi
        bad = ~torch.isfinite(col)
        if bool(bad.any()):
            first = lo + int(torch.nonzero(bad)[0, 0])
            raise FloatingPointError(f"Adam: loss became {float(st['hist'][first, 0])} at epoch {first} "
                                     f"(best finite loss {float(st['best_loss']):.6g} at epoch "
                                     f"{int(st['best_epoch'])}; predict(best_model=True) uses it)")
        return hi


def point_ranges(program, fop):
    from .ops.jet_mlp import hip_config
    spec = os.environ.get("TDQ_SPLIT", "auto").strip().lower()
    if spec in ("0", "off", "none", "", "0.0"):
        return None
    try:
        cfg = hip_config(program.net, program.plan, program.precision)
    except ValueError:
        return None
    if cfg["precision"] not in ("bf16x3", "bf16") or cfg.get("engine") == "layered":
        return None
    from .ops import jet_hip
    if spec == "auto":
        if getattr(program, "hi_op", None) is not None:
            fracs = [0.62]
        else:
            fracs = [0.35] if cfg["precision"] == "bf16x3" else [0.38]
    else:
        fracs = sorted(float(v) for v in spec.split(","))
    if len(fracs) > 1:
        raise ValueError("TDQ_SPLIT: one cut (two point ranges) at most")
    N = program.X_all.shape[0]
    if N < 8192:
        return None
    try:
        pts_b, nwg, chunks, _ = jet_hip.slab_geometry(cfg, N)
        bounds = [(nwg * c // chunks) * pts_b for c in range(1, chunks)]
        bounds = [a for a in bounds if a % 128 == 0]
    except Exception:
        bounds = []
    cuts, blks = [0], [0]
    for f in fracs:
        b = None
        cands = ([min(bounds, key=lambda a: abs(a - f * N))] if bounds else []) + [int(round(f * N / 128)) * 128]
        for a in cands:
            if cuts[-1] < a < N and abs(a - f * N) <= 0.05 * N:
                b = fop.split_block(a)
                if b is not None and b > blks[-1]:
                    break
            b = None
        if b is None:
            return None
        if not cuts[1:] and a < getattr(program, "n_hi", 0) and getattr(program, "hi_op", None) is not None:
            return None
        cuts.append(a)
        blks.append(b)
    cuts.append(N)
    blks.append(fop.n_blocks)
    return [(cuts[i], cuts[i + 1], blks[i], blks[i + 1] - blks[i]) for i in range(len(cuts) - 1)]


def prereduce_chunk(program, ranges):
    if not ranges or len(ranges) != 2 or os.environ.get("TDQ_PREREDUCE", "1") == "0":
        return 0
    from .ops import jet_hip
    from .ops.jet_mlp import hip_config
    cfg = hip_config(program.net, program.plan, program.precision)
    pts_b, nwg, chunks, _ = jet_hip.slab_geometry(cfg, program.X_all.shape[0])
    cut = ranges[0][1]
    for c in range(1, chunks):
        if (nwg * c // chunks) * pts_b == cut:
            return c
    return 0


def run_ranges(program, fop, flat, ranges, streams, pack=True, bufs=None, prereduce=0):
    from .ops import jet_hip
    hop = program.hi_op
    if bufs is None:
        J, saved = jet_hip.alloc_forward(program.X_all, flat, program.net, program.plan, program.precision,
                                         rows=fop.fl.n_streams)
        work = jet_hip.alloc_backward(saved)
    else:
        J, saved, work = bufs
    if pack:
        jet_hip.pack_images(saved)
    if hop is not None and ranges[0][1] < program.n_hi:
        raise RuntimeError("point ranges: the first range must hold the high-order points")
    cur = torch.cuda.current_stream(flat.device)

    def chain(k, lo, hi, b0, nb):
        if k == 0 and hop is not None:
            hop.forward(J, flat)
        jet_hip.forward_range(saved, J, lo, hi)
        fop.run_range(J, b0, nb)
        if k == 0 and hop is not None:
            hop.backward(fop.dJ, flat)
        jet_hip.backward_range(saved, fop.dJ, work, lo, hi)
        if k == 0 and prereduce:
            jet_hip.slab_prereduce(saved, work, 0, prereduce)

    if len(ranges) == 1:
        chain(0, *ranges[0])
        return saved, work
    for st in streams[:len(ranges)]:
        st.wait_stream(cur)
    for k, ((lo, hi, b0, nb), st) in enumerate(zip(ranges, streams)):
        with torch.cuda.stream(st):
            chain(k, lo, hi, b0, nb)
    for st in streams[:len(ranges)]:
        cur.wait_stream(st)
    return saved, work


class PointPass:

    def __init__(self, program, flat, persistent=True):
        self.program, self.flat, self.persistent = program, flat, persistent
        self._bufs, self._ranges, self._streams = None, 0, []
        fop = getattr(program, "fused_op", None)
        self.eligible = False
        if os.environ.get("TDQ_FUSED_TAIL", "1") != "0" and fop is not None and flat.is_cuda:
            from .ops import _lib, jet_hip
            from .ops.jet_mlp import hip_config
            try:
                self.eligible = bool(jet_hip.is_split_bf16(hip_config(program.net, program.plan, program.precision))
                                     and _lib.available())
            except (ValueError, AttributeError):
                pass

    def buffers(self):
        if self._bufs is None:
            from .ops import jet_hip
            prog = self.program
            J, saved = jet_hip.alloc_forward(prog.X_all, self.flat, prog.net, prog.plan, prog.precision,
                                             rows=prog.fused_op.fl.n_streams)
            self._bufs = (J, saved, jet_hip.alloc_backward(saved))
        return self._bufs

    def fused_step(self):
        from .ops import fused_step
        return fused_step.for_program(self.program)

    def ranges(self):
        if self._ranges == 0:
            self._ranges = point_ranges(self.program, self.program.fused_op)
            self._streams = [torch.cuda.Stream(device=self.flat.device) for _ in (self._ranges or ())]
        return self._ranges

    def run(self, pack=True):
        prog, fop = self.program, self.program.fused_op
        fs = self.fused_step()
        if fs is not None:
            J, saved, work = self.buffers()
            fs.run(saved, J, work, self.flat, pack=pack)
            return saved, work, 0, fs.tail_kw()
        rng = self.ranges()
        if not rng and not self.persistent:
            return None
        rng = rng or [(0, prog.X_all.shape[0], 0, fop.n_blocks)]
        pre = prereduce_chunk(prog, rng)
        saved, work = run_ranges(prog, fop, self.flat, rng, self._streams, pack=pack or not self.persistent,
                                 bufs=self.buffers() if self.persistent else None, prereduce=pre)
        return saved, work, pre, {}


class LossGradEngine:

    def __init__(self, solver, program, lambdas):
        self.s = solver
        self.program = program
        self.flat = solver.u_model.flat
        self.lambdas = lambdas
        self.dist = solver.dist_ctx
        self.graph = None
        self.n_evals = 0
        self.points = PointPass(program, self.flat, persistent=False)

    def image_target(self):
        pp = self.points
        if not pp.eligible or getattr(self.program, "hi_op", None) is not None or pp.fused_step() is None:
            return None
        from .ops import jet_hip
        return jet_hip.img_target(pp.buffers()[1]), (lambda: self._body(pack=False))

    def _body(self, pack=True):
        fop = getattr(self.program, "fused_op", None)
        if fop is not None:
            from .ops import jet_hip
            prog = self.program
            if self.points.eligible:
                fg = torch.empty(self.flat.numel() + 1, dtype=torch.float32, device=self.flat.device)
                hi = prog.hi_op
                gx = hi.grad if hi is not None else None
                out = self.points.run(pack)
                if out is not None:
                    saved, work, pre, kw = out
                    jet_hip.dp_tail_a(saved, work, fg[:-1], fop, total=fg[-1:], c_first=pre, gextra=gx, **kw)
                    return fg
                J, saved = jet_hip.forward_raw(prog.X_all, self.flat, prog.net, prog.plan, prog.precision,
                                               rows=fop.fl.n_streams)
                if hi is not None:
                    hi.forward(J, self.flat)
                fop(J, with_total=False, reduce=False)
                if hi is not None:
                    hi.backward(fop.dJ, self.flat)
                grad, work = jet_hip.backward_raw(saved, fop.dJ, reduce=False, grad=fg[:-1])
                jet_hip.dp_tail_a(saved, work, grad, fop, total=fg[-1:], gextra=gx)
                return fg
            hi = prog.hi_op
            J, saved = jet_hip.forward_raw(prog.X_all, self.flat, prog.net, prog.plan, prog.precision,
                                           rows=fop.fl.n_streams)
            if hi is not None:
                hi.forward(J, self.flat)
            total, _, dJ, _, _ = fop(J)
            g = jet_hip.backward_raw(saved, dJ)
            if hi is not None:
                g = g + hi.backward(dJ, self.flat)
            return torch.cat([g.reshape(-1), total.reshape(1)])
        p = self.flat.detach().requires_grad_(True)
        lams = [l.detach() for l in self.lambdas]
        loss, _ = self.program.evaluate(p, lams)
        g = torch.autograd.grad(loss, [p])[0]
        buf = torch.cat([g.reshape(-1), loss.detach().reshape(1)])
        return buf

    def evaluate_fg(self):
        return self._body()

    def __call__(self, x):
        with torch.no_grad():
            self.flat.copy_(x)
        use_graph = _use_graphs(self.flat.device)
        in_graph = self.dist.capturable(self.flat.numel() + 1)
        if use_graph and self.graph is None and self.n_evals >= 1:
            stream = torch.cuda.Stream(device=self.flat.device)
            stream.wait_stream(torch.cuda.current_stream(self.flat.device))
            with torch.cuda.stream(stream):
                self._body()
            torch.cuda.current_stream(self.flat.device).wait_stream(stream)
            g = torch.cuda.CUDAGraph()
            with capture_graph(g):
                self._static = self._body()
                if in_graph:
                    self.dist.all_reduce_(self._static)
            self.graph = g
        if self.graph is not None:
            self.graph.replay()
            buf = self._static.clone()
            reduced = in_graph
        else:
            buf = self._body()
            reduced = False
        self.n_evals += 1
        if self.dist.is_distributed and not reduced:
            self.dist.all_reduce_(buf)
        if in_graph and self.dist.peer is not None and self.n_evals % 32 == 0:
            self.dist.check_health()
        return buf[-1], buf[:-1]


class Timer:
    def __init__(self, device):
        self.device = torch.device(device)

    def sync(self):
        if self.device.type == "cuda":
            torch.cuda.synchronize(self.device)

    def __enter__(self):
        self.sync()
        self.t0 = time.perf_counter()
        return self

    def __exit__(self, *exc):
        self.sync()
        self.elapsed = time.perf_counter() - self.t0
        return False


def nan_guard(loss, where="loss"):
    v = float(loss)
    if math.isnan(v) or math.isinf(v):
        raise FloatingPointError(f"{where} became {v}")
    return v


def fit(obj, tf_iter=0, newton_iter=0, batch_sz=None, newton_eager=True):
    return obj.fit(tf_iter=tf_iter, newton_iter=newton_iter, batch_sz=batch_sz, newton_eager=newton_eager)


def fit_dist(obj, tf_iter=0, newton_iter=0, batch_sz=None, newton_eager=True):
    if not getattr(obj, "dist", False):
        raise ValueError("fit_dist needs a solver compiled with dist=True (launch with torchrun)")
    return obj.fit(tf_iter=tf_iter, newton_iter=newton_iter, batch_sz=batch_sz, newton_eager=newton_eager)


def train_op_inner(obj):
    eng = obj._get_engine(None, 1)
    return eng.run(1, use_graph=False)


def lbfgs_train(obj, newton_iter=100):
    obj._fit_lbfgs(newton_iter, newton_eager=False)
    return obj.min_loss["l-bfgs"]


def lbfgs_op(func, init_params, newton_iter):
    from .optimizers.lbfgs import graph_lbfgs
    return graph_lbfgs(func, init_params, newton_iter)
```

tensordiffeq_amd/ops/_lib.py:

```python
from __future__ import annotations

import ctypes
import os
import threading

import torch

_HERE = os.path.dirname(os.path.abspath(__file__))
LIB_PATH = os.environ.get("TDQ_LIB_PATH") or os.path.join(os.path.dirname(_HERE), "csrc", "libtdq_hip.so")
ABI_VERSION = 27

_lock = threading.Lock()
_lib = None
_err = None


class NativeUnavailable(RuntimeError):
    pass


def _declare(lib):
    c = ctypes
    P, I, F, L, D = c.c_void_p, c.c_int, c.c_float, c.c_int64, c.c_double
    sig = {
        "tdq_abi_version": (I, []),
        "tdq_jet_fwd": (I, [P, P, P, P, I, I, I, I, I, I, P, P]),
        "tdq_jet_bwd": (I, [P, P, P, P, P, P, I, I, I, I, I, I, P, P]),
        "tdq_jet_scratch_floats": (L, [I, I, I, I, I]),
        "tdq_jet_slab_floats": (L, [I, I, I, I, I]),
        "tdq_jet_fwd_bf3": (I, [P, P, P, P, I, I, P, I, I, I, P, I, P]),
        "tdq_jet_bwd_bf3": (I, [P, P, P, P, P, P, I, I, P, I, I, I, P, I, P]),
        "tdq_jet_fwd_bf3_ex": (I, [P, P, P, P, I, I, P, I, I, I, P, I, I, P]),
        "tdq_jet_bwd_bf3_ex": (I, [P, P, P, P, P, P, I, I, P, I, I, I, P, I, I, P]),
        "tdq_jet_fwd_bf3_range": (I, [P, P, P, P, I, I, I, I, P, I, I, I, P, I, I, P]),
        "tdq_jet_bwd_bf3_range": (I, [P, P, P, P, I, I, I, I, P, I, I, I, P, I, P]),
        "tdq_jet_bf3_pack": (I, [P, P, I, I, P, I, I, I, P]),
        "tdq_step_tail_bf3": (I, [P, P, P, I, I, P, I, I, I, I, P, I, I, I, P, P, P] + [P, L, P, P, P, P]
                              + [P, I, P, I, P, I, P, I, P]),
        "tdq_bf3_slab_geometry": (I, [I, I, P, I, I, I, I, P]),
        "tdq_slab_prereduce_bf3": (I, [P, I, I, P, I, I, I, I, I, I, P]),
        "tdq_dp_tail_a_bf3": (I, [P, P, I, I, P, I, I, I, I, P, I, I, I, P, P, P, I, P, I, I, P]),
        "tdq_dp_tail_b_bf3": (I, [P, I, I, P, I, I, I, P, I, P, P, P]),
        "tdq_jet_bf3_scratch_floats": (L, [I, I, P, I, I, I]),
        "tdq_jet_bf3_slab_floats": (L, [I, I, P, I, I]),
        "tdq_fused_step_launch": (I, [P, P, P, P, I, I, P, I, I, I, P, I, P, P, I, I, I, P]),
        "tdq_fused_params_size": (I, []),
        "tdq_jet_fused_lds": (I, [I, P, I, I, I, I]),
        "tdq_device_cus": (I, []),
        "tdq_slab_floats_rows": (L, [I, I, P, I, I]),
        "tdq_lay_nn": (I, [I, P, P, L, P, P, L, P, L, I, I, I, P]),
        "tdq_lay_tn": (I, [I, P, P, L, P, P, L, P, I, I, I, I, P]),
        "tdq_lay_xtz": (I, [P, I, P, I, I, P, I, P]),
        "tdq_lay_xtz2": (I, [P, I, P, P, P, I, I, P, I, P]),
        "tdq_colsum_work": (L, [I, L]),
        "tdq_colsum": (I, [P, L, I, L, P, L, L, L, P, L, I, P, P]),
        "tdq_lay_bplanes": (I, [P, I, I, I, P, P, P]),
        "tdq_lay_l0grad": (I, [P, I, I, P, I, P, P, P]),
        "tdq_lay_nnj": (I, [I, I, I, P, P, P, P, P, I, I, I, P, P, P, P, P, P, P, I, P, P, I, P]),
        "tdq_lay_in_fwd": (I, [I, I, P, P, I, P, P, I, I, P, P, P]),
        "tdq_lay_out_bwd": (I, [I, I, I, P, P, I, P, P, P, I, I, P, P, P, P, I, P]),
        "tdq_adam_multi": (I, [P, I, P, P, P]),
        "tdq_step_book": (I, [P, P, I, I, P, L, P, P, P, P, P, I, P]),
        "tdq_best_track": (I, [P, P, P, P, P, P, L, P]),
        "tdq_loss_fused": (I, [P, P, P, P, P, I, I, I, I, I, I, I, P, P, P, P, I, I, P, P, P, I, I, P]),
        "tdq_loss_fused_range": (I, [P, P, P, P, P, I, I, I, I, I, I, I, P, P, P, P, I, I, I, I, P]),
        "tdq_loss_meta_sizes": (I, [P]),
        "tdq_loss_reduce_partials": (I, [P, I, I, I, P, P, P, I, P]),
        "tdq_lbfgs_nst": (I, []),
        "tdq_lbfgs_ticket_ints": (I, []),
        "tdq_lbfgs_update": (I, [P] * 14 + [I] * 6 + [D] * 4 + [I, P]),
        "tdq_lbfgs_axpy": (I, [P, P, P, I, I, P]),
        "tdq_lbfgs_update_fused": (I, [P] * 16 + [I] * 6 + [D] * 4 + [I, P, P]),
        "tdq_img_target": (I, [P, I, P, I, I, P, I]),
        "tdq_layered_epi": (I, [I, P, P, P, L, I, I, P, P, P, P, P, P]),
        "tdq_jet_hi_scratch_floats": (L, [I, I]),
        "tdq_jet_hi_work_floats": (L, [I, I, P, I, I]),
        "tdq_jet_hi_fwd": (I, [P, I, P, I, P, I, I, P, P, P, I, I, P, P]),
        "tdq_jet_hi_bwd": (I, [P, I, P, I, P, I, I, P, P, P, I, I, P, P, P, P]),
        "tdq_jet_hi_bwd_part": (I, [P, I, P, I, P, I, I, P, P, P, I, I, P, P, P, I, P]),
        "tdq_jet_hi_limits": (I, [P]),
        "tdq_jet_hi_lds_ok": (I, [I, I, I, I]),
        "tdq_jet_hi_tile_ok": (I, [I, I, I, I, I, I]),
        "tdq_jet_hi_tile_scratch_floats": (L, [I, I, I]),
        "tdq_jet_hi_tile_work_floats": (L, [I, I, P, I, I, I]),
        "tdq_jet_hi_tile_fwd": (I, [P, I, P, I, P, I, I, P, P, P, I, I, P, I, P]),
        "tdq_jet_hi_tile_bwd_part": (I, [P, I, P, I, P, I, I, P, P, P, I, I, P, P, P, I, I, P]),
        "tdq_peer_maxw": (I, []),
        "tdq_peer_chunk": (I, []),
        "tdq_peer_alloc": (I, [L, I, P]),
        "tdq_peer_free": (I, [P]),
        "tdq_peer_ipc_handle": (I, [P, P]),
        "tdq_peer_ipc_open": (I, [P, P]),
        "tdq_peer_ipc_close": (I, [P]),
        "tdq_peer_allreduce": (I, [P, I, I, I, L, I, P, P, P, P, L, P]),
        "tdq_rtc_compile": (I, [c.c_char_p, c.c_char_p, c.c_char_p, P, P, c.c_char_p, I]),
        "tdq_rtc_compile_ex": (I, [c.c_char_p, c.c_char_p, c.c_char_p, c.c_char_p, P, P, c.c_char_p, I]),
        "tdq_rtc_free": (None, [P]),
        "tdq_rtc_load": (I, [P, c.c_char_p, P, P]),
        "tdq_rtc_unload": (I, [P]),
        "tdq_rtc_set_global_ptr": (I, [P, c.c_char_p, P]),
        "tdq_loss_jit_range": (I, [P, P, P, P, P, P, I, I, P]),
    }
    for name, (res, args) in sig.items():
        fn = getattr(lib, name, None)
        if fn is None:
            continue
        fn.restype = res
        fn.argtypes = args


def load(required=None):
    global _lib, _err
    with _lock:
        if _lib is not None:
            return _lib
        if _err is not None and not required:
            raise NativeUnavailable(_err)
        if not os.path.exists(LIB_PATH):
            _err = f"{LIB_PATH} not built (run `python -m tensordiffeq_amd.csrc.build`)"
            raise NativeUnavailable(_err)
        try:
            lib = ctypes.CDLL(LIB_PATH)
            _declare(lib)
            ver = lib.tdq_abi_version()
            if ver != ABI_VERSION:
                _err = f"libtdq_hip.so ABI {ver} != expected {ABI_VERSION}; rebuild"
                raise NativeUnavailable(_err)
            built, want = library_hash(lib), expected_hash()
            if want is not None and built != want and os.environ.get("TDQ_SKIP_HASH_CHECK", "0") != "1":
                _err = (f"{LIB_PATH} is stale: built from sources {built}, the csrc/ sources hash to {want} "
                        f"(run `python -m tensordiffeq_amd.csrc.build`)")
                raise NativeUnavailable(_err)
        except OSError as e:
            _err = f"cannot load {LIB_PATH}: {e}"
            raise NativeUnavailable(_err)
        _lib = lib
        return _lib


def library_hash(lib):
    fn = getattr(lib, "tdq_src_hash", None)
    if fn is None:
        return None
    fn.restype = ctypes.c_char_p
    fn.argtypes = []
    return fn().decode()


def expected_hash():
    from ..csrc import build as _build
    if not _build.source_files():
        return None
    return _build.source_hash()


def available():
    try:
        load()
        return True
    except NativeUnavailable:
        return False


def fallback_allowed():
    return os.environ.get("TDQ_ALLOW_TORCH_FALLBACK", "0") == "1"


def gpu_present():
    try:
        return torch.cuda.is_available()
    except Exception:
        return False


def require_on_gpu():
    if gpu_present() and not fallback_allowed():
        load(required=True)


def stream_ptr(device=None):
    return ctypes.c_void_p(torch.cuda.current_stream(device).cuda_stream)


def check(rc, what):
    if rc != 0:
        raise RuntimeError(f"{what} failed with HIP error {rc}")


def ptr(t):
    return ctypes.c_void_p(t.data_ptr()) if t is not None else ctypes.c_void_p(0)
```

tensordiffeq_amd/ops/fused_step.py:

```python
from __future__ import annotations

import collections
import ctypes
import hashlib
import os
import warnings

import torch

from . import _lib, jet_hip, loss_jit
from .jet_mlp import hip_config

_CACHE = {}
_HEADERS = ("common.h", "jet_common.h", "jet_bf3.h", "jet_fused.h", "jet_fused3.h")
RTC_OPTS = "-O3 -std=c++17 -fno-slp-vectorize -munsafe-fp-atomics"


RTC_OPTS_LO = " -mllvm -amdgpu-sched-strategy=max-ilp -DTDQ_COL4_BPERMUTE"


def _opts(src=""):
    extra = os.environ.get("TDQ_FUSED_STEP_DEFINES", "")
    return RTC_OPTS + (RTC_OPTS_LO if "fz3_body<" in src else "") + \
        (" -DTDQ_PHASE_TIMING" if os.environ.get("TDQ_FUSED_STEP_TIMING") == "1" else "") + \
        (" " + extra if extra else "")


def enabled():
    return os.environ.get("TDQ_FUSED_STEP", "1") != "0"


def systems_enabled():
    return os.environ.get("TDQ_FUSED_STEP_SYSTEMS", "1") != "0"


def _csrc():
    return os.path.join(os.path.dirname(os.path.dirname(os.path.abspath(__file__))), "csrc")


def header_source():
    out = []
    for h in _HEADERS:
        with open(os.path.join(_csrc(), h)) as f:
            lines = f.read().splitlines()
        out.append("\n".join(ln for ln in lines if not ln.strip().startswith('#include "')
                             and ln.strip() != "#pragma once"))
    return "\n".join(out)


def spec_source(spec, S, d_in, d_out=1):
    if spec is None or d_in is None:
        raise ValueError("gen_loss: the stream spec and d_in are compile-time constants of the kernel")
    M = 8
    st, var, ia, ib = [0] * M, [0] * M, [0] * M, [0] * M
    selA = [[0.0] * M for _ in range(M)]
    selB = [[0.0] * M for _ in range(M)]
    for s in range(S):
        ty, a, b = spec[3 * s:3 * s + 3]
        st[s] = ty
        if ty == 1:
            var[s] = a
        if ty == 2:
            ia[s], ib[s] = a, b
            selA[s][a] = 1.0
            selB[s][b] = 1.0
    arr = lambda v: "{" + ", ".join(str(x) for x in v) + "}"
    mat = lambda m: "{" + ", ".join("{" + ", ".join(f"{x:.1f}f" for x in r) + "}" for r in m) + "}"
    return [f"  static constexpr JetSpec SPEC = {{{arr(st)}, {arr(var)}, {mat(selA)}, {mat(selB)}, {arr(ia)}, "
            f"{arr(ib)}}};",
            f"  static constexpr int DIN = {int(d_in)};",
            f"  static constexpr int DOUT = {int(d_out)};"]


def gen_loss(groups, n_terms, nacc, S, spec=None, d_in=None, d_out=1):
    D = int(d_out)
    if not 1 <= D <= 4:
        raise ValueError(f"fused step: {D} network outputs")
    cmask = (1 << loss_jit.COL_SHIFT) - 1

    def dj(sl, s, q):
        return f"dj{sl}_{s}" + (f"_{q}" if D > 1 else "")

    def jv(s, k, q):
        return f"JV({s}, {k}" + (f", {q})" if D > 1 else ")")

    def ub(s, k, q):
        return f"UB({s}, {k}" + (f", {q})" if D > 1 else ")")

    L = []
    e = L.append
    e("struct GenLoss {")
    e(f"  static constexpr int NACC = {max(1, nacc)};")
    for ln in spec_source(spec, S, d_in, D):
        e(ln)

    def branches(body):
        kw = "if"
        for (P, start, ns, n) in groups:
            end = start + ns * n
            e(f"    {kw} (n >= {start} && n < {end} && n < N) {{")
            kw = "else if"
            if ns == 2:
                e(f"      if ((n - {start}) & 1) return;   // the pair's first point-thread owns it")
                e(f"      const int i = (n - {start}) >> 1;")
            else:
                e(f"      const int i = n - {start};")
            body(P, ns)
            e("      return;")
            e("    }")

    first = {}
    for gi, (P, start, ns, n) in enumerate(groups):
        seen = []

        def probe(name, r, a, b, seen=seen):
            if name in ("VAL", "LAM") and not seen:
                seen.append((name, a))
            return ""
        loss_jit._forward_code(P, lambda _ln: None, probe)
        first[gi] = seen[0] if seen else None
    e("  __device__ static float pre(int n, int N, const FzLossPtrs& ptr) {")
    kw = "if"
    for gi, (P, start, ns, n) in enumerate(groups):
        if first[gi] is None:
            continue
        nm, a = first[gi]
        arr = {"VAL": "val", "LAM": "lam"}[nm]
        end = start + ns * n
        idx = f"(n - {start}) >> 1" if ns == 2 else f"n - {start}"
        e(f"    {kw} (n >= {start} && n < {end} && n < N) return ptr.{arr}[{a}][{idx}];")
        kw = "else if"
    e("    return 0.f;")
    e("  }")
    e("  template <int S, int PT, int NW>")
    e("  __device__ static void eval(const float* jv, const float* xs, int t, int n, int N, "
      "const FzLossPtrs& ptr, float* ubs, float (&acc)[NACC], float pv, "
      + ("float bo" if D == 1 else "const float* bo") + ") {")
    if D == 1:
        e("    #define JV(s_, k_) fz_jsum<S, PT, NW>(jv, (s_), (k_), bo)")
        e("    #define UB(s_, k_) ubs[((s_) * PT + (k_)) * 4]")
    else:
        e(f"    #define JV(s_, k_, q_) fz_jsum_q<S, PT, NW, {D}>(jv, (s_), (k_), (q_), bo)")
        e("    #define UB(s_, k_, q_) ubs[((s_) * PT + (k_)) * 4 + (q_)]")

    cur = {}

    def eval_body(P, ns):
        fp = first[[g[0] for g in groups].index(P)]
        cur["first"], cur["used"] = fp, False
        nr = max(1, P.n_regs)
        e("      float " + ", ".join(f"v{r}" for r in range(nr)) + ";")
        e("      float " + ", ".join(f"a{r} = 0.f" for r in range(nr)) + ";")
        e("      float " + ", ".join(f"{dj(sl, b, q)} = 0.f" for sl in range(ns) for b in range(S)
                                     for q in range(D)) + ";")

        def stream(b):
            s, q = b & cmask, b >> loss_jit.COL_SHIFT
            if s >= S or q >= D:
                raise ValueError("fused step: stream outside the jet plan")
            return s, q

        def load(name, r, a, b):
            if name in ("STREAM", "COORD") and a >= ns:
                raise ValueError("fused step: slot outside the group")
            if name == "STREAM":
                s, q = stream(b)
                return f"      v{r} = {jv(s, f't + {a}', q)};"
            if name == "COORD":
                return f"      v{r} = xs[(t + {a}) * TDQ_MAXD + {b}];"
            if (name, a) == cur["first"] and not cur["used"]:
                cur["used"] = True
                return f"      v{r} = pv;   // prefetched (pre)"
            return {"VAL": f"      v{r} = ptr.val[{a}][i];", "LAM": f"      v{r} = ptr.lam[{a}][i];",
                    "SCAL": f"      v{r} = *ptr.scal[{a}];"}[name]

        loss_jit._forward_code(P, e, load)
        for (f, w, tt, c) in P.outputs:
            cl = loss_jit._lit(c)
            e(f"      {{ const float f = v{f}, w = v{w};")
            e(f"        acc[{tt}] += {cl} * w * f * f;")
            e(f"        a{f} += 2.f * {cl} * w * f; a{w} += {cl} * f * f; }}")

        def store(name, r, a, b, g):
            if name == "STREAM":
                return f"      {dj(a, *stream(b))} += {g};"
            if name == "LAM":
                return f"      ptr.dlam[{a}][i] = {g};"
            return f"      acc[{n_terms + a}] += {g};"

        loss_jit._reverse_code(P, e, store)
        rows = [" ".join(f"{ub(b, f't + {sl}', q)} = {dj(sl, b, q)};" for q in range(D))
                for sl in range(ns) for b in range(S)]
        for ln in ([" ".join(rows)] if D == 1 else rows):
            e("      " + ln)

    branches(eval_body)
    e("    #pragma unroll")
    zero = " ".join(f"{ub('s', 't', q)} = 0.f;" for q in range(D))
    e("    for (int s = 0; s < S; ++s) " + (zero if D == 1 else "{ " + zero + " }"))
    e("    #undef JV")
    e("    #undef UB")
    e("  }")
    e("};")
    return "\n".join(L)


def kernel_name(lo=False):
    return "tdq_fused_step3" if lo else "tdq_fused_step"


def kernel_source(S, nso, LM, lds, gen, lo=False):
    body = "fz3_body" if lo else "fz_body"
    return (header_source() + "\n" + gen + "\n"
            'extern "C" __global__ void __launch_bounds__(64 * FZ_WAVES) '
            f"__attribute__((amdgpu_waves_per_eu(2, 2))) {kernel_name(lo)}(FzParams P) {{\n"
            f"  __shared__ __attribute__((aligned(16))) char lds[{lds}];\n"
            f"  {body}<8, {S}, {nso}, {LM}, GenLoss>(P, lds);\n"
            "}\n")


_PENDING = {}


def _key(src):
    return hashlib.sha256((loss_jit.device_arch() + _opts(src) + src).encode()).hexdigest()


def _rtc_compile(src):
    lib = _lib.load(required=True)
    code, size = ctypes.c_void_p(0), ctypes.c_longlong(0)
    log = ctypes.create_string_buffer(16384)
    rc = lib.tdq_rtc_compile_ex(src.encode(), b"tdq_fused_step.hip", loss_jit.device_arch().encode(),
                                _opts(src).encode(), ctypes.byref(code), ctypes.byref(size), log, len(log))
    if rc != 0:
        raise RuntimeError(f"hipRTC compile failed ({rc}): {log.value.decode(errors='replace')[:2000]}")
    try:
        return ctypes.string_at(code, size.value)
    finally:
        lib.tdq_rtc_free(code)


def compile_async(src):
    import threading
    k = _key(src)
    if k in _CACHE or k in _PENDING:
        return
    out = []

    def work():
        try:
            out.append(_rtc_compile(src))
        except Exception as e:
            out.append(e)
    th = threading.Thread(target=work, name="tdq-rtc", daemon=True)
    _PENDING[k] = (th, out)
    th.start()


def _compile(src, name="tdq_fused_step"):
    lib = _lib.load(required=True)
    k = _key(src)
    if k not in _CACHE:
        pend = _PENDING.pop(k, None)
        if pend is not None:
            pend[0].join()
            code = pend[1][0]
            if isinstance(code, Exception):
                raise code
        else:
            code = _rtc_compile(src)
        buf = ctypes.create_string_buffer(code, len(code))
        mod, fn = ctypes.c_void_p(0), ctypes.c_void_p(0)
        _lib.check(lib.tdq_rtc_load(buf, name.encode(), ctypes.byref(mod), ctypes.byref(fn)), "hipModuleLoadData")
        _CACHE[k] = (mod, fn)
    return _CACHE[k]


def mixed_mode():
    mode = os.environ.get("TDQ_FUSED_STEP_MIXED", "split")
    if mode not in ("split", "0"):
        raise ValueError(f"TDQ_FUSED_STEP_MIXED={mode!r}: accepted values are 'split' and '0'")
    return mode


def _mixed(prog):
    return getattr(prog, "hi_op", None) is not None


def fused_groups(prog, fop):
    from .. import fusion
    out = []
    for gr in fop.fl.groups:
        if all(s < prog.plan.S for (_, s) in gr.program.stream_regs):
            out.append((gr, gr.program, None))
            continue
        sp = fusion.split_by_streams(fop.fl, gr, prog.plan.S)
        if sp is None:
            return "a loss output reads main-plan and high-order streams together (or both read one SA weight)"
        out.append((gr, sp[0], sp[1]))
    return out


def point_layout(prog, groups):
    layout, idx = [], []
    for gr, P_f, _ in groups:
        ns = len(gr.segs)
        if ns == 2 and len(idx) % 2:
            idx.append(-1)
        layout.append((P_f, len(idx), ns, gr.n))
        offs = [prog.segments[sg].offset for sg in gr.segs]
        for k in range(gr.n):
            idx.extend(o + k for o in offs)
    return layout, idx, len(idx)


KernelRecipe = collections.namedtuple("KernelRecipe", "cfg S spec nso LM lo pt lds name source")


def recipe(prog, fop, layout, precision=None):
    cfg = hip_config(prog.net, prog.plan, precision or prog.precision)
    S = cfg["S"]
    spec = jet_hip.stream_spec(prog.plan)
    nso = sum(1 for s in range(S) if spec[3 * s] == 2)
    LM = cfg["n_hidden"] - 1
    lo = cfg["precision"] == "bf16x3"
    lds = _lib.load(required=True).tdq_jet_fused_lds(cfg["d_in"], jet_hip._warg(cfg), cfg["d_out"], cfg["n_hidden"],
                                                     S, int(lo))
    if lds < 0 or lds > 160 * 1024:
        raise ValueError(f"fused step: {lds} bytes of LDS")
    source = None
    if layout is not None:
        gen = gen_loss(layout, fop.n_terms, fop.n_terms + fop.n_scal, S, spec=spec, d_in=cfg["d_in"],
                       d_out=cfg["d_out"])
        source = kernel_source(S, nso, LM, lds, gen, lo=lo)
    return KernelRecipe(cfg, S, spec, nso, LM, lo, 16 if lo else 32, lds, kernel_name(lo), source)


def program_recipe(prog, fop, precision=None):
    groups = fused_groups(prog, fop)
    if isinstance(groups, str):
        raise ValueError(groups)
    layout, idx, N = point_layout(prog, groups)
    return recipe(prog, fop, layout, precision), groups, idx, N


def prebuild(prog):
    if not torch.cuda.is_available():
        return False
    fop = getattr(prog, "fused_op", None)
    if ineligible(prog, fop) is not None or _mixed(prog):
        return False
    compile_async(program_recipe(prog, fop)[0].source)
    return True


def ineligible(prog, fop):
    if not enabled():
        return "TDQ_FUSED_STEP=0"
    mode = mixed_mode()
    if prog.device.type != "cuda" or fop is None:
        return "needs the fused loss on a GPU"
    try:
        cfg = hip_config(prog.net, prog.plan, prog.precision)
    except ValueError as e:
        return str(e)
    if cfg["precision"] not in ("bf16", "bf16x3") or not jet_hip.is_split_bf16(cfg):
        return f"precision {cfg['precision']}"
    if cfg["d_out"] != 1:
        if not (systems_enabled() and cfg["d_out"] <= 4 and not _mixed(prog) and cfg["S"] <= 4
                and cfg["n_hidden"] - 1 in (2, 3) and all(w == 128 for w in cfg["widths"])):
            return "d_out != 1"
        try:
            recipe(prog, fop, None)
        except ValueError as e:
            return f"LDS: {e} ({cfg['precision']}, {cfg['n_hidden']} hidden layers, S={cfg['S']}, d_out={cfg['d_out']})"
    try:
        recipe(prog, fop, None)
    except ValueError:
        return f"network {cfg['widths']} / S={cfg['S']} (width-128 MFMA layers 2-3, S <= 4)"
    if not _mixed(prog):
        if any(s >= cfg["S"] for gr in fop.fl.groups for (_, s) in gr.program.stream_regs):
            return "a loss group reads streams outside the jet plan"
        return None
    if cfg["precision"] == "bf16x3":
        return "bf16x3: high-order boundary streams keep the separate launches"
    if mode == "0":
        return "high-order boundary streams (TDQ_FUSED_STEP_MIXED=0)"
    sp = fused_groups(prog, fop)
    return sp if isinstance(sp, str) else None


class FusedStepOp:

    def __init__(self, prog, fop):
        lib = _lib.load(required=True)
        self.prog, self.fop = prog, fop
        rec, groups, idx, self.N = program_recipe(prog, fop)
        cfg = self.cfg = rec.cfg
        self.lo, self.pt, self.lds, self.source = rec.lo, rec.pt, rec.lds, rec.source
        self.nacc = fop.n_terms + fop.n_scal
        dev = prog.device
        self.mixed = _mixed(prog)
        self.layout = "split" if self.mixed else "plain"
        ix = torch.tensor(idx, dtype=torch.long, device=dev)
        X_f = prog.X_all[ix.clamp_min(0)].clone()
        X_f[ix < 0] = 0.0
        self.X = X_f.contiguous()
        self.fop2, self.prow = None, 0
        if self.mixed:
            import copy
            from ..fusion import Group
            from .loss_fused import FusedLossOp
            fl2 = copy.copy(fop.fl)
            fl2.groups = []
            for gr, _, P_s in groups:
                if P_s is not None:
                    g2 = Group(list(gr.segs), gr.n)
                    g2.program = P_s
                    fl2.groups.append(g2)
            self.fop2 = FusedLossOp(fl2, prog, fop.lams, fop.scalars, fop.fl.lam_offsets)
            self.fop2.ptrs = fop.ptrs
            self.prow = self.fop2.n_blocks
        self.module, self.func = _compile(self.source, rec.name)
        ntiles = -(-self.N // self.pt)
        cus = max(1, lib.tdq_device_cus())
        rounds = -(-ntiles // cus)
        if self.fop2 is not None:
            rounds += int(os.environ.get("TDQ_FS_SPLIT_ROUNDS", "1" if rounds <= 16 else "0"))
        self.G = -(-ntiles // rounds)
        self.free_cus = cus - self.G
        need = lib.tdq_slab_floats_rows(self.G, cfg["d_in"], jet_hip._warg(cfg), cfg["d_out"], cfg["n_hidden"])
        cap = lib.tdq_jet_bf3_slab_floats(prog.X_all.shape[0], cfg["d_in"], jet_hip._warg(cfg), cfg["d_out"],
                                          cfg["n_hidden"])
        if need < 0 or need > cap:
            raise ValueError(f"fused step: {self.G} slab rows do not fit the backward's buffer")
        self.n_lblocks = self.prow + self.G
        self.lpart = torch.zeros(max(1, self.n_lblocks * self.nacc), dtype=torch.float32, device=dev)
        self._side = None
        if self.fop2 is not None:
            self.fop2.partials = self.lpart[:self.prow * self.nacc]
            self._side = torch.cuda.Stream(device=dev)

    def run(self, saved, J, work, flat, pack=True):
        lib = _lib.load()
        fop, cfg = self.fop, self.cfg
        if pack:
            jet_hip.pack_images(saved)
        cur = torch.cuda.current_stream(flat.device)
        side = self._side
        hop = self.prog.hi_op
        _, _, scratch, _, spec, S = saved
        spec_arr = (ctypes.c_int * len(spec))(*spec)

        def fused():
            rc = lib.tdq_fused_step_launch(self.func, _lib.ptr(self.X), _lib.ptr(scratch), _lib.ptr(work), self.N,
                                           cfg["d_in"], jet_hip._warg(cfg), cfg["d_out"], cfg["n_hidden"], S,
                                           spec_arr, self.G, _lib.ptr(fop.ptrs), _lib.ptr(self.lpart),
                                           self.prow, self.nacc, int(self.lo), _lib.stream_ptr(flat.device))
            _lib.check(rc, "tdq_fused_step_launch")

        if side is None:
            fused()
            return
        order = os.environ.get("TDQ_FS_SPLIT_ORDER", "fused_first" if self.free_cus >= 32 else "side_first")
        ev = torch.cuda.Event()
        ev.record(cur)
        if order != "side_first":
            fused()
        side.wait_event(ev)
        with torch.cuda.stream(side):
            hop.forward(J, flat)
            self.fop2.run_range(J, 0, self.fop2.n_blocks)
            hop.backward(self.fop2.dJ, flat)
        if order == "side_first":
            fused()
        cur.wait_stream(side)

    def set_timing_buffer(self, buf):
        _lib.check(_lib.load().tdq_rtc_set_global_ptr(self.module, b"tdq_ts", ctypes.c_void_p(buf.data_ptr())),
                   "tdq_rtc_set_global_ptr")

    def tail_kw(self):
        return {"rows": self.G, "lpart": self.lpart, "n_lblocks": self.n_lblocks}


def for_program(prog):
    if getattr(prog, "_fused_step_built", False):
        return prog._fused_step
    if torch.cuda.is_available() and torch.cuda.is_current_stream_capturing():
        warnings.warn("fused training step first requested inside a graph capture; using separate launches")
        return None
    prog._fused_step_built = True
    prog._fused_step = None
    fop = getattr(prog, "fused_op", None)
    why = ineligible(prog, fop)
    if why is None:
        try:
            prog._fused_step = FusedStepOp(prog, fop)
        except Exception as e:
            why = f"{type(e).__name__}: {e}"
            warnings.warn(f"fused training step unavailable, using separate launches: {why}")
    prog.fused_step_reason = why
    return prog._fused_step
```

tensordiffeq_amd/ops/jet_hip.py:

```python
from __future__ import annotations

import ctypes

import torch

from . import _lib
from .jet_mlp import hip_config


def stream_spec(plan):
    idx = plan.index
    out = []
    for mi in plan.streams:
        if len(mi) == 0:
            out += [0, 0, 0]
        elif len(mi) == 1:
            out += [1, mi[0], 0]
        else:
            out += [2, idx[(mi[0],)], idx[(mi[1],)]]
    return out


def _warg(cfg):
    if cfg["precision"] in ("bf16x3", "bf16"):
        w = cfg["widths"]
        return (ctypes.c_int * len(w))(*w)
    return cfg["width"]


def _fns(lib, cfg):
    if cfg["precision"] in ("bf16x3", "bf16"):
        return (lib.tdq_jet_fwd_bf3, lib.tdq_jet_bwd_bf3,
                lambda N: lib.tdq_jet_bf3_scratch_floats(N, cfg["d_in"], _warg(cfg), cfg["n_hidden"], cfg["S"],
                                                         *_lo_args(cfg)),
                lambda N: lib.tdq_jet_bf3_slab_floats(N, cfg["d_in"], _warg(cfg), cfg["d_out"], cfg["n_hidden"]))
    return (lib.tdq_jet_fwd, lib.tdq_jet_bwd,
            lambda N: lib.tdq_jet_scratch_floats(N, cfg["width"], cfg["n_hidden"], cfg["S"], 0),
            lambda N: lib.tdq_jet_slab_floats(N, cfg["d_in"], cfg["width"], cfg["d_out"], cfg["n_hidden"]))


def _lo_args(cfg):
    if cfg["precision"] == "bf16x3":
        return (1,)
    if cfg["precision"] == "bf16":
        return (0,)
    return ()


def forward_raw(X, P, net, plan, precision=None, pack=True, rows=None):
    lib = _lib.load()
    cfg = hip_config(net, plan, precision)
    if is_layered(cfg):
        from . import jet_layered
        return jet_layered.forward_raw(X.contiguous(), P, net, plan, cfg["precision"])
    fwd, _, scratch_floats, _ = _fns(lib, cfg)
    X = X.contiguous()
    N = X.shape[0]
    S = plan.S
    spec = stream_spec(plan)
    spec_c = (ctypes.c_int * len(spec))(*spec)
    J = torch.empty((max(S, rows or S), N, cfg["d_out"]), dtype=torch.float32, device=X.device)
    nscr = scratch_floats(N)
    if nscr < 0:
        raise ValueError(f"jet kernels cannot serve {cfg}")
    scratch = torch.empty(max(int(nscr), 1), dtype=torch.float32, device=X.device)
    if not pack and cfg["precision"] in ("bf16x3", "bf16"):
        rc = lib.tdq_jet_fwd_bf3_ex(_lib.ptr(X), _lib.ptr(P), _lib.ptr(J), _lib.ptr(scratch), N, cfg["d_in"],
                                    _warg(cfg), cfg["d_out"], cfg["n_hidden"], S, spec_c, *_lo_args(cfg), 0,
                                    _lib.stream_ptr(X.device))
    else:
        rc = fwd(_lib.ptr(X), _lib.ptr(P), _lib.ptr(J), _lib.ptr(scratch), N, cfg["d_in"],
                 _warg(cfg), cfg["d_out"], cfg["n_hidden"], S, spec_c, *_lo_args(cfg), _lib.stream_ptr(X.device))
    _lib.check(rc, f"tdq_jet_fwd[{cfg['precision']}]")
    return J, (X, P, scratch, cfg, spec, S)


def backward_raw(saved, dJ, reduce=True, grad=None):
    if saved[0] == "layered":
        if not reduce:
            raise ValueError("backward_raw(reduce=False) needs the fused split-bf16 kernels")
        from . import jet_layered
        return jet_layered.backward_raw(saved, dJ, grad=grad)
    lib = _lib.load()
    X, P, scratch, cfg, spec, S = saved
    _, bwd, _, slab_floats = _fns(lib, cfg)
    N = X.shape[0]
    dJ = dJ.contiguous()
    nwork = slab_floats(N)
    work = torch.empty(max(int(nwork), 1), dtype=torch.float32, device=X.device)
    if grad is None:
        grad = torch.empty_like(P)
    spec_c = (ctypes.c_int * len(spec))(*spec)
    if not reduce:
        if not is_split_bf16(cfg):
            raise ValueError("backward_raw(reduce=False) needs a split-bf16 precision")
        rc = lib.tdq_jet_bwd_bf3_ex(_lib.ptr(X), _lib.ptr(P), _lib.ptr(dJ), _lib.ptr(scratch), _lib.ptr(work),
                                    _lib.ptr(grad), N, cfg["d_in"], _warg(cfg), cfg["d_out"], cfg["n_hidden"],
                                    S, spec_c, *_lo_args(cfg), 0, _lib.stream_ptr(X.device))
        _lib.check(rc, f"tdq_jet_bwd_bf3_ex[{cfg['precision']}]")
        return grad, work
    rc = bwd(_lib.ptr(X), _lib.ptr(P), _lib.ptr(dJ), _lib.ptr(scratch), _lib.ptr(work),
                         _lib.ptr(grad), N, cfg["d_in"], _warg(cfg), cfg["d_out"], cfg["n_hidden"], S,
                         spec_c, *_lo_args(cfg), _lib.stream_ptr(X.device))
    _lib.check(rc, f"tdq_jet_bwd[{cfg['precision']}]")
    return grad


def alloc_forward(X, P, net, plan, precision=None, rows=None):
    cfg = hip_config(net, plan, precision)
    if not is_split_bf16(cfg):
        raise ValueError("point-range launches need a split-bf16 precision")
    lib = _lib.load()
    _, _, scratch_floats, _ = _fns(lib, cfg)
    X = X.contiguous()
    N = X.shape[0]
    nscr = scratch_floats(N)
    if nscr < 0:
        raise ValueError(f"jet kernels cannot serve {cfg}")
    J = torch.empty((max(plan.S, rows or plan.S), N, cfg["d_out"]), dtype=torch.float32, device=X.device)
    scratch = torch.empty(max(int(nscr), 1), dtype=torch.float32, device=X.device)
    return J, (X, P, scratch, cfg, stream_spec(plan), plan.S)


def forward_range(saved, J, lo, hi):
    lib = _lib.load()
    X, P, scratch, cfg, spec, S = saved
    spec_c = (ctypes.c_int * len(spec))(*spec)
    rc = lib.tdq_jet_fwd_bf3_range(_lib.ptr(X), _lib.ptr(P), _lib.ptr(J), _lib.ptr(scratch), X.shape[0], int(lo),
                                   int(hi), cfg["d_in"], _warg(cfg), cfg["d_out"], cfg["n_hidden"], S, spec_c,
                                   *_lo_args(cfg), 0, _lib.stream_ptr(X.device))
    _lib.check(rc, "tdq_jet_fwd_bf3_range")


def alloc_backward(saved):
    lib = _lib.load()
    X, P, scratch, cfg, spec, S = saved
    _, _, _, slab_floats = _fns(lib, cfg)
    return torch.empty(max(int(slab_floats(X.shape[0])), 1), dtype=torch.float32, device=X.device)


def backward_range(saved, dJ, work, lo, hi):
    lib = _lib.load()
    X, P, scratch, cfg, spec, S = saved
    spec_c = (ctypes.c_int * len(spec))(*spec)
    rc = lib.tdq_jet_bwd_bf3_range(_lib.ptr(X), _lib.ptr(dJ), _lib.ptr(scratch), _lib.ptr(work), X.shape[0],
                                   int(lo), int(hi), cfg["d_in"], _warg(cfg), cfg["d_out"], cfg["n_hidden"], S,
                                   spec_c, *_lo_args(cfg), _lib.stream_ptr(X.device))
    _lib.check(rc, "tdq_jet_bwd_bf3_range")


def is_split_bf16(cfg):
    return cfg["precision"] in ("bf16x3", "bf16") and not is_layered(cfg)


def is_layered(cfg):
    return cfg.get("engine") == "layered"


def pack_images(saved):
    lib = _lib.load()
    X, P, scratch, cfg, spec, S = saved
    rc = lib.tdq_jet_bf3_pack(_lib.ptr(P), _lib.ptr(scratch), X.shape[0], cfg["d_in"], _warg(cfg),
                              cfg["d_out"], cfg["n_hidden"], S, _lib.stream_ptr(X.device))
    _lib.check(rc, "tdq_jet_bf3_pack")


def img_target(saved):
    lib = _lib.load()
    X, P, scratch, cfg, spec, S = saved
    buf = ctypes.create_string_buffer(256)
    rc = lib.tdq_img_target(_lib.ptr(scratch), cfg["d_in"], _warg(cfg), cfg["d_out"], cfg["n_hidden"], buf, 256)
    if rc <= 0:
        raise RuntimeError("tdq_img_target: unsupported network")
    return buf


def slab_geometry(cfg, N):
    lib = _lib.load()
    out = (ctypes.c_int * 4)()
    rc = lib.tdq_bf3_slab_geometry(int(N), cfg["d_in"], _warg(cfg), cfg["d_out"], cfg["n_hidden"], cfg["S"],
                                   *_lo_args(cfg), out)
    _lib.check(rc, "tdq_bf3_slab_geometry")
    return tuple(out)


def slab_prereduce(saved, work, c0, c1):
    lib = _lib.load()
    X, P, scratch, cfg, spec, S = saved
    rc = lib.tdq_slab_prereduce_bf3(_lib.ptr(work), X.shape[0], cfg["d_in"], _warg(cfg), cfg["d_out"],
                                    cfg["n_hidden"], S, *_lo_args(cfg), int(c0), int(c1), _lib.stream_ptr(X.device))
    _lib.check(rc, "tdq_slab_prereduce_bf3")


def step_tail(saved, work, grad, fop, book, counters, group_array, n_groups, snapshot, write_images=True,
              c_first=0, gextra=None, rows=0, lpart=None, n_lblocks=None):
    lib = _lib.load()
    X, P, scratch, cfg, spec, S = saved
    hist = book["hist"]
    carr = (ctypes.c_void_p * max(1, len(counters)))(*[c.data_ptr() for c in counters])
    rc = lib.tdq_step_tail_bf3(
        _lib.ptr(work), _lib.ptr(grad), _lib.ptr(scratch) if write_images else None,
        X.shape[0], cfg["d_in"], _warg(cfg), cfg["d_out"], cfg["n_hidden"], S, *_lo_args(cfg),
        _lib.ptr(fop.partials if lpart is None else lpart), fop.n_blocks if n_lblocks is None else int(n_lblocks),
        fop.n_terms, fop.n_scal,
        _lib.ptr(fop.losses), _lib.ptr(fop.total), _lib.ptr(fop.dscal),
        _lib.ptr(hist), int(hist.shape[0]), _lib.ptr(book["epoch"]), _lib.ptr(book["best_loss"]),
        _lib.ptr(book["best_epoch"]), _lib.ptr(book["improved"]), ctypes.cast(carr, ctypes.c_void_p), len(counters),
        ctypes.cast(group_array, ctypes.c_void_p), n_groups,
        _lib.ptr(snapshot) if snapshot is not None else None, int(c_first), _lib.ptr(gextra), int(rows),
        _lib.stream_ptr(X.device))
    _lib.check(rc, "tdq_step_tail_bf3")


class JetMLPFunction(torch.autograd.Function):
    @staticmethod
    def forward(ctx, X, params, net, plan, precision=None):
        J, saved = forward_raw(X, params.contiguous(), net, plan, precision)
        if saved[0] == "layered":
            ctx.layered = saved
            return J
        ctx.layered = None
        ctx.save_for_backward(saved[0], saved[1], saved[2])
        ctx.meta = saved[3:]
        return J

    @staticmethod
    def backward(ctx, dJ):
        if ctx.layered is not None:
            saved = ctx.layered
            if dJ is None:
                dJ = torch.zeros((len(saved[4]) // 3, saved[1].shape[0], saved[3].layer_sizes[-1]),
                                 device=saved[1].device)
            return None, backward_raw(saved, dJ), None, None, None
        X, P, scratch = ctx.saved_tensors
        cfg, spec, S = ctx.meta
        if dJ is None:
            dJ = torch.zeros((S, X.shape[0], cfg["d_out"]), device=X.device)
        return None, backward_raw((X, P, scratch, cfg, spec, S), dJ), None, None, None


def dp_tail_a(saved, work, grad, fop, total=None, losses=None, c_first=0, gextra=None, rows=0, lpart=None,
              n_lblocks=None, half=None):
    lib = _lib.load()
    X, P, scratch, cfg, spec, S = saved
    losses = fop.losses if losses is None else losses
    rc = lib.tdq_dp_tail_a_bf3(_lib.ptr(work), _lib.ptr(grad), X.shape[0], cfg["d_in"], _warg(cfg), cfg["d_out"],
                               cfg["n_hidden"], S, *_lo_args(cfg), _lib.ptr(fop.partials if lpart is None else lpart),
                               fop.n_blocks if n_lblocks is None else int(n_lblocks), fop.n_terms,
                               fop.n_scal, _lib.ptr(losses), _lib.ptr(fop.dscal), _lib.ptr(total), int(c_first),
                               _lib.ptr(gextra), int(rows), -1 if half is None else int(bool(half)),
                               _lib.stream_ptr(X.device))
    _lib.check(rc, "tdq_dp_tail_a_bf3")


def dp_tail_b(saved, group_array, n_groups, improved, snapshot):
    lib = _lib.load()
    X, P, scratch, cfg, spec, S = saved
    rc = lib.tdq_dp_tail_b_bf3(_lib.ptr(scratch), X.shape[0], cfg["d_in"], _warg(cfg), cfg["d_out"],
                               cfg["n_hidden"], S, ctypes.cast(group_array, ctypes.c_void_p), n_groups,
                               _lib.ptr(improved), _lib.ptr(snapshot), _lib.stream_ptr(X.device))
    _lib.check(rc, "tdq_dp_tail_b_bf3")
```

Measured before the change: 374.4 million collocation-pts/s.

## Fuse step tail reduction, loss bookkeeping and Adam into one launch

Replaces the two-kernel step tail (slab reduce plus separate Adam kernel) with a single kernel. Each block reduces its slab chunks in LDS, computes the loss total and learning rates locally, and applies Adam in place. Counter and best-loss bookkeeping is moved into a pre-book structure consumed by the fused step kernel. The snapshot decision now compares against a previous best-loss copy, so no cross-kernel dependency is needed. This removes a launch and a global partial-sum round trip per step, at the cost of redundant per-block loss-slot sums and stricter eligibility conditions.

```diff
diff --git a/tensordiffeq_amd/csrc/jet_bf3.hip b/tensordiffeq_amd/csrc/jet_bf3.hip
--- a/tensordiffeq_amd/csrc/jet_bf3.hip
+++ b/tensordiffeq_amd/csrc/jet_bf3.hip
@@ -1,5 +1,9 @@
+#include <cstdlib>
+
 #include "jet_fused3.h"
 #include "optim_common.h"
+
+static_assert(FZ_MAX_COUNTERS == TDQ_MAX_COUNTERS, "FzPreBook holds every step counter");
 
 __device__ __forceinline__ void pack_frag(const float* __restrict__ P, bf16x8* __restrict__ img, const NetDims& d,
                                           int WT, int transposed, int e) {
@@ -80,6 +84,26 @@
   Counters cnt;
 };
 
+__device__ __forceinline__ void tail_book_block(const TailBook& tb, bool bump) {
+  if (threadIdx.x >= 64) return;
+  const int ns = tb.n_terms + tb.n_scal;
+  for (int slot = 0; slot < ns; ++slot) {
+    const float s = loss_slot_sum(tb.lpart, tb.n_lblocks, ns, slot, threadIdx.x);
+    if (threadIdx.x == 0) {
+      if (slot < tb.n_terms) tb.losses[slot] = s;
+      else tb.dscal[slot - tb.n_terms] = s;
+    }
+  }
+  if (threadIdx.x == 0 && tb.hist == nullptr && tb.total != nullptr) {
+    float s = 0.f;
+    for (int t = 0; t < tb.n_terms; ++t) s += tb.losses[t];
+    *tb.total = s;
+  }
+  if (threadIdx.x == 0 && tb.hist != nullptr)
+    step_book_body(tb.total, tb.losses, tb.n_terms, 1, tb.hist, tb.hist_rows, tb.epoch, tb.best_loss, tb.best_epoch,
+                   tb.improved, tb.cnt, bump);
+}
+
 __global__ void __launch_bounds__(256) tail_reduce1_kernel(const float* __restrict__ slab, float* __restrict__ part,
                                                            int nwg, int Pst, int chunks, int nqb, int half, int c0,
                                                            TailBook tb) {
@@ -93,31 +117,7 @@
     return;
   }
   if (blockIdx.y != 0) return;
-  __shared__ float sh[256];
-  const int ns = tb.n_terms + tb.n_scal;
-  for (int slot = 0; slot < ns; ++slot) {
-    float s = 0.f;
-    for (int b = threadIdx.x; b < tb.n_lblocks; b += 256) s += tb.lpart[(size_t)b * ns + slot];
-    sh[threadIdx.x] = s;
-    __syncthreads();
-    for (int k = 128; k > 0; k >>= 1) {
-      if ((int)threadIdx.x < k) sh[threadIdx.x] += sh[threadIdx.x + k];
-      __syncthreads();
-    }
-    if (threadIdx.x == 0) {
-      if (slot < tb.n_terms) tb.losses[slot] = sh[0];
-      else tb.dscal[slot - tb.n_terms] = sh[0];
-    }
-    __syncthreads();
-  }
-  if (threadIdx.x == 0 && tb.hist == nullptr && tb.total != nullptr) {
-    float s = 0.f;
-    for (int t = 0; t < tb.n_terms; ++t) s += tb.losses[t];
-    *tb.total = s;
-  }
-  if (threadIdx.x == 0 && tb.hist != nullptr)
-    step_book_body(tb.total, tb.losses, tb.n_terms, 1, tb.hist, tb.hist_rows, tb.epoch, tb.best_loss, tb.best_epoch,
-                   tb.improved, tb.cnt);
+  tail_book_block(tb, true);
 }
 
 __global__ void __launch_bounds__(256) slab_reduce2_bf3(const float* __restrict__ part, float* __restrict__ grad, int P,
@@ -128,6 +128,17 @@
 #pragma unroll
   for (int e = 0; e < 4; ++e)
     if (4 * q + e < P) grad[4 * q + e] = gx != nullptr ? a[e] + gx[4 * q + e] : a[e];
+}
+
+__device__ __forceinline__ void tail_adam_elem(const AdamGroup& gr, int64_t e, float p, float m, float v, float g,
+                                               float lr_t, bool th, bool do_snap, float* __restrict__ snap,
+                                               const TailImg& ti) {
+  if (do_snap && th) snap[e] = p;
+  adam_elem(p, gr.sign * g, m, v, gr.b1, gr.b2, gr.eps, lr_t);
+  gr.p[e] = p;
+  gr.m[e] = m;
+  gr.v[e] = v;
+  if (th && ti.fimg != nullptr) scatter_param(p, (int)e, ti);
 }
 
 __global__ void __launch_bounds__(256) tail_adam_kernel(AdamArgs args, const float* __restrict__ part, int Pst,
@@ -143,37 +154,124 @@
     const bool th = gi == 0;
     float g;
     if (th && part != nullptr) {
-      float a0 = 0.f, a1 = 0.f;
-      int c = 0;
-      for (; c + 7 < chunks; c += 8) {
-        float v[8];
-#pragma unroll
-        for (int k = 0; k < 8; ++k) v[k] = part[(size_t)(c + k) * Pst + e];
-#pragma unroll
-        for (int k = 0; k < 8; k += 2) {
-          a0 += v[k];
-          a1 += v[k + 1];
-        }
-      }
-      for (; c + 1 < chunks; c += 2) {
-        a0 += part[(size_t)c * Pst + e];
-        a1 += part[(size_t)(c + 1) * Pst + e];
-      }
-      if (c < chunks) a0 += part[(size_t)c * Pst + e];
-      g = a0 + a1;
+      g = slab_part_sum(part + e, (size_t)Pst, chunks);
       if (gx != nullptr) g += gx[e];
       const_cast<float*>(gr.g)[e] = g;
     } else {
       g = gr.g[e];
     }
-    float p = gr.p[e], m = gr.m[e], v = gr.v[e];
-    if (do_snap && th) snap[e] = p;
-    adam_elem(p, gr.sign * g, m, v, gr.b1, gr.b2, gr.eps, adam_lr_t(gr));
-    gr.p[e] = p;
-    gr.m[e] = m;
-    gr.v[e] = v;
-    if (th && ti.fimg != nullptr) scatter_param(p, (int)e, ti);
-  }
+    tail_adam_elem(gr, e, gr.p[e], gr.m[e], gr.v[e], g, adam_lr_t(gr), th, do_snap, snap, ti);
+  }
+}
+
+#define TAIL1_MAX_SLOTS 64
+#define TAIL1_CHUNKS 8
+
+template <bool H>
+__device__ __forceinline__ void tail_one_partials(const void* __restrict__ slab, float* __restrict__ sp, int nwg,
+                                                  int Pst, int chunks, int cb, int tid) {
+  if constexpr (H) {
+    const int cg = tid & 31, c = tid >> 5, q8 = cb * 32 + cg;
+    if (8 * q8 < Pst && c < chunks) {
+      f32x4 s_lo, s_hi;
+      slab_chunk_sum8(slab, nwg, Pst, chunks, q8, c, s_lo, s_hi);
+      f32x4* o = reinterpret_cast<f32x4*>(sp + c * 256 + 8 * cg);
+      o[0] = s_lo;
+      o[1] = s_hi;
+    }
+  } else {
+    const int cq = tid & 63, q = cb * 64 + cq;
+    if (4 * q < Pst)
+      for (int c = tid >> 6; c < chunks; c += 4)
+        *reinterpret_cast<f32x4*>(sp + c * 256 + 4 * cq) = slab_chunk_sum<false>(slab, nwg, Pst, chunks, q, c);
+  }
+}
+
+struct TailOne {
+  const void* slab;
+  int nwg, Pst, P, chunks;
+  int ncb;
+  float* grad;
+  const float* gx;
+};
+
+template <bool H>
+__global__ void __launch_bounds__(256) tail_one_reduce_kernel(TailOne t, TailBook tb) {
+  __shared__ __attribute__((aligned(16))) float sp[TAIL1_CHUNKS * 256];
+  const int cb = blockIdx.x, tid = threadIdx.x;
+  if (cb >= t.ncb) {
+    tail_book_block(tb, true);
+    return;
+  }
+  tail_one_partials<H>(t.slab, sp, t.nwg, t.Pst, t.chunks, cb, tid);
+  __syncthreads();
+  const int e = cb * 256 + tid;
+  if (e < t.P) {
+    const float g = slab_part_sum(sp + tid, (size_t)256, t.chunks);
+    t.grad[e] = t.gx != nullptr ? g + t.gx[e] : g;
+  }
+}
+
+template <bool H>
+__global__ void __launch_bounds__(256) tail_one_kernel(TailOne t, TailBook tb, AdamArgs args,
+                                                       const float* __restrict__ best_prev,
+                                                       float* __restrict__ snap, TailImg ti) {
+  __shared__ __attribute__((aligned(16))) float sp[TAIL1_CHUNKS * 256];
+  __shared__ float s_lr[TDQ_MAX_GROUPS];
+  __shared__ float s_ls[TAIL1_MAX_SLOTS];
+  __shared__ float s_total;
+  const int cb = blockIdx.x, tid = threadIdx.x;
+  const int nob = (int)gridDim.x - 1 - t.ncb;
+  if (cb >= t.ncb + nob) {
+    tail_book_block(tb, false);
+    return;
+  }
+  const bool th = cb < t.ncb;
+  int gi = 0;
+  int64_t e = (int64_t)cb * 256 + tid;
+  bool live = e < t.P;
+  if (!th) {
+    const int64_t idx = args.start[1] + (int64_t)(cb - t.ncb) * 256 + tid;
+    live = idx < args.start[args.ngroups];
+    gi = live ? adam_group_of(args, idx) : 0;
+    e = idx - args.start[gi];
+  }
+  const AdamGroup gr = args.grp[gi];
+  float p = 0.f, m = 0.f, v = 0.f;
+  if (live) {
+    p = gr.p[e];
+    m = gr.m[e];
+    v = gr.v[e];
+  }
+  const int ns = tb.n_terms + tb.n_scal;
+  if (tid >= 192) {
+    if (tid - 192 < args.ngroups) s_lr[tid - 192] = adam_lr_t(args.grp[tid - 192]);
+  } else if (tid >= 128) {
+    for (int slot = 0; slot < ns; ++slot) {
+      const float s = loss_slot_sum(tb.lpart, tb.n_lblocks, ns, slot, tid - 128);
+      if (tid == 128) s_ls[slot] = s;
+    }
+    if (tid == 128) {
+      float lv = 0.f;
+      for (int k = 0; k < tb.n_terms; ++k) lv += s_ls[k];
+      s_total = lv;
+    }
+  }
+  if (th) tail_one_partials<H>(t.slab, sp, t.nwg, t.Pst, t.chunks, cb, tid);
+  __syncthreads();
+  if (!live) return;
+  float g;
+  if (th) {
+    g = slab_part_sum(sp + tid, (size_t)256, t.chunks);
+    if (t.gx != nullptr) g += t.gx[e];
+    t.grad[e] = g;
+  } else if (tb.n_scal > 0 && gr.g >= tb.dscal && gr.g + gr.n <= tb.dscal + tb.n_scal) {
+    g = s_ls[tb.n_terms + (int)(gr.g - tb.dscal) + (int)e];
+  } else {
+    g = gr.g[e];
+  }
+  const bool do_snap = snap != nullptr && s_total < *best_prev;
+  tail_adam_elem(gr, e, p, m, v, g, s_lr[gi], th, do_snap, snap, ti);
 }
 
 namespace {
@@ -206,6 +304,11 @@
 bool bf3_ok(int WT, int S, int d_in, int d_out, int n_hidden) {
   return (WT == 2 || WT == 4 || WT == 8 || (WT == 16 && S <= 4)) && S >= 1 && S <= TDQ_MAXS &&
          d_in <= TDQ_MAXD && d_out <= TDQ_MAXO && n_hidden >= 1;
+}
+
+bool tail_one_enabled() {
+  const char* v = getenv("TDQ_TAIL_ONE");
+  return v == nullptr || v[0] != '0' || v[1] != '\0';
 }
 
 int dispatch(bool fwd, int WT, int S, int nso, const Bf3Args& a) {
@@ -359,11 +462,12 @@
   return tdq_jet_bwd_bf3_ex(X, P, dJ, Hs, work, grad, N, d_in, widths, d_out, n_hidden, S, spec, lo, 1, stream);
 }
 
-int tdq_step_tail_bf3(float* work, float* grad, float* scratch, int N, int d_in, const int* widths, int d_out, int n_hidden,
-                      int S, int lo, const float* lpart, int n_lblocks, int n_terms, int n_scal, float* losses,
-                      float* total, float* dscal, float* hist, int64_t hist_rows, int64_t* epoch, float* best_loss,
-                      int64_t* best_epoch, int* improved, double* const* counters, int ncnt, const void* groups,
-                      int ngroups, float* snap, int c_first, const float* gx, int rows, void* stream) {
+static int step_tail_launch(float* work, float* grad, float* scratch, int N, int d_in, const int* widths, int d_out,
+                            int n_hidden, int S, int lo, const float* lpart, int n_lblocks, int n_terms, int n_scal,
+                            float* losses, float* total, float* dscal, float* hist, int64_t hist_rows, int64_t* epoch,
+                            float* best_loss, int64_t* best_epoch, int* improved, double* const* counters, int ncnt,
+                            const void* groups, int ngroups, float* snap, int c_first, const float* gx, int rows,
+                            const float* best_prev, void* stream) {
   NetDims d;
   if (!make_dims(d, d_in, widths, 0, d_out, n_hidden)) return (int)hipErrorInvalidValue;
   const int WT = width_tiles(d.width);
@@ -399,9 +503,6 @@
   for (int i = 0; i < TDQ_MAX_COUNTERS; ++i) tb.cnt.c[i] = i < ncnt ? counters[i] : nullptr;
   const int half = (int)slab_half(lo != 0);
   const int nqb = (Pst / (half ? 8 : 4) + 255) / 256;
-  hipLaunchKernelGGL(tail_reduce1_kernel, dim3(nqb + 1, chunks - c_first), dim3(256), 0, st, work, part, nwg_b, Pst,
-                     chunks, nqb, half, c_first, tb);
-  TDQ_CHECK_LAUNCH();
   TailImg ti{nullptr, nullptr, nullptr, d, WT};
   if (scratch != nullptr) {
     float *img, *bimg, *aux;
@@ -411,6 +512,23 @@
     ti.aux = aux;
   }
   const int64_t tot = args.start[ngroups];
+  if (best_prev != nullptr) {
+    const int64_t nob = (tot - args.start[1] + 255) / 256;
+    if (c_first != 0 || chunks > TAIL1_CHUNKS || n_terms + n_scal > TAIL1_MAX_SLOTS || hist == nullptr ||
+        nob > (1 << 30))
+      return (int)hipErrorInvalidValue;
+    const TailOne t{work, nwg_b, Pst, Ptot, chunks, (Pst + 255) / 256, grad, gx};
+    const dim3 grid((unsigned)(t.ncb + nob + 1));
+    if (half)
+      hipLaunchKernelGGL(tail_one_kernel<true>, grid, dim3(256), 0, st, t, tb, args, best_prev, snap, ti);
+    else
+      hipLaunchKernelGGL(tail_one_kernel<false>, grid, dim3(256), 0, st, t, tb, args, best_prev, snap, ti);
+    TDQ_CHECK_LAUNCH();
+    return 0;
+  }
+  hipLaunchKernelGGL(tail_reduce1_kernel, dim3(nqb + 1, chunks - c_first), dim3(256), 0, st, work, part, nwg_b, Pst,
+                     chunks, nqb, half, c_first, tb);
+  TDQ_CHECK_LAUNCH();
   int64_t blocks = (tot + 255) / 256;
   if (blocks > 2048) blocks = 2048;
   if (blocks < 1) blocks = 1;
@@ -419,6 +537,38 @@
   TDQ_CHECK_LAUNCH();
   return 0;
 }
+
+int tdq_step_tail_bf3(float* work, float* grad, float* scratch, int N, int d_in, const int* widths, int d_out, int n_hidden,
+                      int S, int lo, const float* lpart, int n_lblocks, int n_terms, int n_scal, float* losses,
+                      float* total, float* dscal, float* hist, int64_t hist_rows, int64_t* epoch, float* best_loss,
+                      int64_t* best_epoch, int* improved, double* const* counters, int ncnt, const void* groups,
+                      int ngroups, float* snap, int c_first, const float* gx, int rows, void* stream) {
+  return step_tail_launch(work, grad, scratch, N, d_in, widths, d_out, n_hidden, S, lo, lpart, n_lblocks, n_terms,
+                          n_scal, losses, total, dscal, hist, hist_rows, epoch, best_loss, best_epoch, improved,
+                          counters, ncnt, groups, ngroups, snap, c_first, gx, rows, nullptr, stream);
+}
+
+int tdq_step_tail1_bf3(float* work, float* grad, float* scratch, int N, int d_in, const int* widths, int d_out,
+                       int n_hidden, int S, int lo, const float* lpart, int n_lblocks, int n_terms, int n_scal,
+                       float* losses, float* total, float* dscal, float* hist, int64_t hist_rows, int64_t* epoch,
+                       float* best_loss, int64_t* best_epoch, int* improved, double* const* counters, int ncnt,
+                       const void* groups, int ngroups, float* snap, int c_first, const float* gx, int rows,
+                       const float* best_prev, void* stream) {
+  if (best_prev == nullptr) return (int)hipErrorInvalidValue;
+  return step_tail_launch(work, grad, scratch, N, d_in, widths, d_out, n_hidden, S, lo, lpart, n_lblocks, n_terms,
+                          n_scal, losses, total, dscal, hist, hist_rows, epoch, best_loss, best_epoch, improved,
+                          counters, ncnt, groups, ngroups, snap, c_first, gx, rows, best_prev, stream);
+}
+
+__global__ void step_prebook_kernel(const FzPreBook* __restrict__ pre) { step_prebook(pre); }
+int tdq_step_prebook(const void* pre, void* stream) {
+  if (pre == nullptr) return (int)hipErrorInvalidValue;
+  hipLaunchKernelGGL(step_prebook_kernel, dim3(1), dim3(1), 0, reinterpret_cast<hipStream_t>(stream),
+                     reinterpret_cast<const FzPreBook*>(pre));
+  TDQ_CHECK_LAUNCH();
+  return 0;
+}
+int tdq_prebook_size() { return (int)sizeof(FzPreBook); }
 
 int tdq_dp_tail_a_bf3(float* work, float* grad, int N, int d_in, const int* widths, int d_out, int n_hidden, int S, int lo,
                       const float* lpart, int n_lblocks, int n_terms, int n_scal, float* losses, float* dscal,
@@ -442,8 +592,16 @@
   tb.losses = losses;
   tb.dscal = dscal;
   tb.total = total;
-  const int half = half_ovr >= 0 ? (half_ovr != 0) : (int)slab_half(lo != 0);
+  const int half = half_ovr >= 0 ? (half_ovr == 1) : (int)slab_half(lo != 0);
+  const bool one = half ? tail_one_enabled() : half_ovr == 2;
   const int nqb = (Pst / (half ? 8 : 4) + 255) / 256, nq2 = (Pst / 4 + 255) / 256;
+  if (c_first == 0 && chunks <= TAIL1_CHUNKS && one) {
+    const TailOne t{work, nwg_b, Pst, Ptot, chunks, (Pst + 255) / 256, grad, gx};
+    if (half) hipLaunchKernelGGL(tail_one_reduce_kernel<true>, dim3(t.ncb + 1), dim3(256), 0, st, t, tb);
+    else hipLaunchKernelGGL(tail_one_reduce_kernel<false>, dim3(t.ncb + 1), dim3(256), 0, st, t, tb);
+    TDQ_CHECK_LAUNCH();
+    return 0;
+  }
   hipLaunchKernelGGL(tail_reduce1_kernel, dim3(nqb + 1, chunks - c_first), dim3(256), 0, st, work, part, nwg_b, Pst,
                      chunks, nqb, half, c_first, tb);
   TDQ_CHECK_LAUNCH();
@@ -516,8 +674,8 @@
 
 int tdq_fused_step_launch(void* func, const float* X, float* scratch, float* work, int N, int d_in, const int* widths,
                           int d_out, int n_hidden, int S, const int* spec, int G, const void* lptrs,
-                          float* lpart, int prow, int nacc, int lo, void* stream) {
-  if (func == nullptr || N <= 0 || G < 1 || prow < 0 || nacc < 1 || lo < 0 || lo > 1)
+                          float* lpart, int prow, int nacc, int lo, const void* pre, void* stream) {
+  if (func == nullptr || N <= 0 || G < 1 || prow < 0 || nacc < 1 || lo < 0 || lo > 1 || (lo && pre != nullptr))
     return (int)hipErrorInvalidValue;
   NetDims d;
   if (!make_dims(d, d_in, widths, 0, d_out, n_hidden)) return (int)hipErrorInvalidValue;
@@ -544,6 +702,7 @@
   P.lpart = lpart;
   P.prow = prow;
   P.nacc = nacc;
+  P.pre = reinterpret_cast<const FzPreBook*>(pre);
   void* args[] = {(void*)&P};
   return (int)hipModuleLaunchKernel((hipFunction_t)func, (unsigned)G, 1, 1, 64 * FZ_WAVES, 1, 1, 0,
                                     reinterpret_cast<hipStream_t>(stream), args, nullptr);
diff --git a/tensordiffeq_amd/csrc/jet_common.h b/tensordiffeq_amd/csrc/jet_common.h
--- a/tensordiffeq_amd/csrc/jet_common.h
+++ b/tensordiffeq_amd/csrc/jet_common.h
@@ -132,10 +132,9 @@
 }
 
 template <bool H = false>
-__device__ __forceinline__ void slab_reduce1_body(const void* __restrict__ slab, float* __restrict__ part, int nwg,
-                                                  int Pst, int chunks, int q, int c) {
+__device__ __forceinline__ f32x4 slab_chunk_sum(const void* __restrict__ slab, int nwg, int Pst, int chunks, int q,
+                                                int c) {
   const int lo = slab_chunk_lo(nwg, chunks, c), hi = slab_chunk_lo(nwg, chunks, c + 1);
-  const size_t row = (size_t)(Pst >> 2);
   f32x4 a0 = zero4(), a1 = zero4(), a2 = zero4(), a3 = zero4();
   int wgi = lo;
   for (; wgi + 3 < hi; wgi += 4) {
@@ -145,7 +144,12 @@
     a3 += slab_ld4<H>(slab, wgi + 3, Pst, q);
   }
   for (; wgi < hi; ++wgi) a0 += slab_ld4<H>(slab, wgi, Pst, q);
-  reinterpret_cast<f32x4*>(part)[(size_t)c * row + q] = (a0 + a1) + (a2 + a3);
+  return (a0 + a1) + (a2 + a3);
+}
+template <bool H = false>
+__device__ __forceinline__ void slab_reduce1_body(const void* __restrict__ slab, float* __restrict__ part, int nwg,
+                                                  int Pst, int chunks, int q, int c) {
+  reinterpret_cast<f32x4*>(part)[(size_t)c * (size_t)(Pst >> 2) + q] = slab_chunk_sum<H>(slab, nwg, Pst, chunks, q, c);
 }
 
 __device__ __forceinline__ void bf8_add(f32x4& lo, f32x4& hi, const uint4 u) {
@@ -154,8 +158,8 @@
   hi += f32x4{__uint_as_float(u.z << 16), __uint_as_float(u.z & 0xffff0000u), __uint_as_float(u.w << 16),
               __uint_as_float(u.w & 0xffff0000u)};
 }
-__device__ __forceinline__ void slab_reduce1_body8(const void* __restrict__ slab, float* __restrict__ part, int nwg,
-                                                   int Pst, int chunks, int q8, int c) {
+__device__ __forceinline__ void slab_chunk_sum8(const void* __restrict__ slab, int nwg, int Pst, int chunks, int q8,
+                                                int c, f32x4& s_lo, f32x4& s_hi) {
   const int lo = slab_chunk_lo(nwg, chunks, c), hi = slab_chunk_lo(nwg, chunks, c + 1);
   const uint4* s8 = reinterpret_cast<const uint4*>(slab) + q8;
   const size_t rs = (size_t)(Pst >> 3);
@@ -184,20 +188,23 @@
     bf8_add(a3, b3, u3);
   }
   for (; w < hi; ++w) bf8_add(a0, b0, s8[(size_t)w * rs]);
+  s_lo = (a0 + a1) + (a2 + a3);
+  s_hi = (b0 + b1) + (b2 + b3);
+}
+__device__ __forceinline__ void slab_reduce1_body8(const void* __restrict__ slab, float* __restrict__ part, int nwg,
+                                                   int Pst, int chunks, int q8, int c) {
   f32x4* p4 = reinterpret_cast<f32x4*>(part) + (size_t)c * (size_t)(Pst >> 2) + 2 * q8;
-  p4[0] = (a0 + a1) + (a2 + a3);
-  p4[1] = (b0 + b1) + (b2 + b3);
-}
-
-__device__ __forceinline__ f32x4 slab_reduce2_sum(const float* __restrict__ part, int Pst, int chunks, int q) {
-  const f32x4* p4 = reinterpret_cast<const f32x4*>(part) + q;
-  const size_t row = (size_t)(Pst >> 2);
-  f32x4 a0 = zero4(), a1 = zero4();
+  slab_chunk_sum8(slab, nwg, Pst, chunks, q8, c, p4[0], p4[1]);
+}
+
+template <class T>
+__device__ __forceinline__ T slab_part_sum(const T* __restrict__ p, size_t stride, int chunks) {
+  T a0 = T{}, a1 = T{};
   int c = 0;
   for (; c + 7 < chunks; c += 8) {
-    f32x4 v[8];
+    T v[8];
 #pragma unroll
-    for (int k = 0; k < 8; ++k) v[k] = p4[(size_t)(c + k) * row];
+    for (int k = 0; k < 8; ++k) v[k] = p[(size_t)(c + k) * stride];
 #pragma unroll
     for (int k = 0; k < 8; k += 2) {
       a0 += v[k];
@@ -205,11 +212,14 @@
     }
   }
   for (; c + 1 < chunks; c += 2) {
-    a0 += p4[(size_t)c * row];
-    a1 += p4[(size_t)(c + 1) * row];
-  }
-  if (c < chunks) a0 += p4[(size_t)c * row];
+    a0 += p[(size_t)c * stride];
+    a1 += p[(size_t)(c + 1) * stride];
+  }
+  if (c < chunks) a0 += p[(size_t)c * stride];
   return a0 + a1;
+}
+__device__ __forceinline__ f32x4 slab_reduce2_sum(const float* __restrict__ part, int Pst, int chunks, int q) {
+  return slab_part_sum(reinterpret_cast<const f32x4*>(part) + q, (size_t)(Pst >> 2), chunks);
 }
 
 extern "C" int tdq_slab_reduce(float* work, float* grad, int nwg, int P, int chunks, void* stream);
diff --git a/tensordiffeq_amd/csrc/jet_fused.h b/tensordiffeq_amd/csrc/jet_fused.h
--- a/tensordiffeq_amd/csrc/jet_fused.h
+++ b/tensordiffeq_amd/csrc/jet_fused.h
@@ -205,6 +205,19 @@
   const float* scal[8];
 };
 
+#define FZ_MAX_COUNTERS 8
+struct FzPreBook {
+  double* c[FZ_MAX_COUNTERS];
+  int n, pad;
+  const float* best_loss;
+  float* best_prev;
+};
+__device__ __forceinline__ void step_prebook(const FzPreBook* __restrict__ pb) {
+  const int n = pb->n;
+  for (int i = 0; i < n && i < FZ_MAX_COUNTERS; ++i) *pb->c[i] += 1.0;
+  *pb->best_prev = *pb->best_loss;
+}
+
 struct FzParams {
   const float* X;
   const float* aux;
@@ -216,6 +229,7 @@
   const FzLossPtrs* lptrs;
   float* lpart;
   int prow, nacc;
+  const FzPreBook* pre;
 };
 
 template <int S, int PT, int NW>
@@ -313,6 +327,7 @@
     }
   };
   if (t0 < t1) fetch(t0);
+  if (P.pre != nullptr && gi == 0 && tid == 0) step_prebook(P.pre);
   fz_setup<WT, LM, F.xs>(P, aux, tid);
   f32x4 dk[LM][NR][NC];
   float lacc[LossF::NACC];
diff --git a/tensordiffeq_amd/csrc/optim.hip b/tensordiffeq_amd/csrc/optim.hip
--- a/tensordiffeq_amd/csrc/optim.hip
+++ b/tensordiffeq_amd/csrc/optim.hip
@@ -67,7 +67,7 @@
 
 extern "C" {
 
-int tdq_abi_version() { return 27; }
+int tdq_abi_version() { return 28; }
 
 int tdq_step_book(float* loss, const float* terms, int n_terms, int sum_terms, float* hist, int64_t hist_rows,
                   int64_t* epoch, float* best_loss, int64_t* best_epoch, int* improved, double* const* counters,
diff --git a/tensordiffeq_amd/csrc/optim_common.h b/tensordiffeq_amd/csrc/optim_common.h
--- a/tensordiffeq_amd/csrc/optim_common.h
+++ b/tensordiffeq_amd/csrc/optim_common.h
@@ -67,7 +67,7 @@
                                                int n_terms, int sum_terms, float* __restrict__ hist,
                                                int64_t hist_rows, int64_t* __restrict__ epoch,
                                                float* __restrict__ best_loss, int64_t* __restrict__ best_epoch,
-                                               int* __restrict__ improved, const Counters& cnt) {
+                                               int* __restrict__ improved, const Counters& cnt, bool bump = true) {
   float lv = *loss;
   if (sum_terms) {
     lv = 0.f;
@@ -86,6 +86,22 @@
     *best_epoch = ep;
   }
   *improved = imp;
-  for (int i = 0; i < cnt.n; ++i) *cnt.c[i] += 1.0;
+  if (bump)
+    for (int i = 0; i < cnt.n; ++i) *cnt.c[i] += 1.0;
   *epoch = ep + 1;
 }
+
+__device__ __forceinline__ float loss_slot_sum(const float* __restrict__ lpart, int n_rows, int ns, int slot,
+                                               int lane) {
+  float leaf[4];
+#pragma unroll
+  for (int k = 0; k < 4; ++k) {
+    float s = 0.f;
+    for (int b = lane + 64 * k; b < n_rows; b += 256) s += lpart[(size_t)b * ns + slot];
+    leaf[k] = s;
+  }
+  float y = (leaf[0] + leaf[2]) + (leaf[1] + leaf[3]);
+#pragma unroll
+  for (int k = 32; k > 0; k >>= 1) y += __shfl_down(y, k, 64);
+  return y;
+}
diff --git a/tensordiffeq_amd/fit.py b/tensordiffeq_amd/fit.py
--- a/tensordiffeq_amd/fit.py
+++ b/tensordiffeq_amd/fit.py
@@ -72,6 +72,8 @@
         self.points = PointPass(program, self.flat)
         self._fsrc = self._grad = self._dp_buf = self._sig = self.graph_k = self._graph_saved = None
         self._sum_terms = False
+        self._prebook_key = self._prebook_dev = self._best_prev = None
+        self.tail_launches = 0
         self._bind_opts()
         self._ensure_hist(n_steps_hint)
 
@@ -225,7 +227,8 @@
         if st["best_flat"].numel() != self.flat.numel():
             raise ValueError(f"best-weights snapshot has {st['best_flat'].numel()} elements, parameters "
                              f"{self.flat.numel()}")
-        saved, work, pre, kw = self.points.run(pack=not in_graph)
+        one = self._tail_one()
+        saved, work, pre, kw = self.points.run(pack=not in_graph, prebook=self._prebook() if one else None)
         if self._grad is None:
             self._grad = torch.empty_like(self.flat)
         grad = self._grad
@@ -236,9 +239,29 @@
                                "(set TDQ_FUSED_TAIL=0)")
         hi = prog.hi_op
         jet_hip.step_tail(saved, work, grad, fop, st, self.counters, packed[0], packed[1], st["best_flat"],
-                          write_images=in_graph, c_first=pre, gextra=hi.grad if hi is not None else None, **kw)
+                          write_images=in_graph, c_first=pre, gextra=hi.grad if hi is not None else None,
+                          best_prev=self._best_prev if one else None, **kw)
         self._tail_saved = saved
+        self.tail_launches = 1 if one else 2
         return fop.total
+
+    def _tail_one(self):
+        from .ops import jet_hip
+        fs = self.points.fused_step()
+        return (jet_hip.tail_one_enabled() and not self.dist.is_distributed and fs is not None and not fs.lo
+                and fs.layout in ("plain", "split") and fs.fop.n_terms + fs.fop.n_scal <= 64
+                and len(self.counters) <= 8)
+
+    def _prebook(self):
+        from .ops import jet_hip
+        st = self.state
+        key = tuple(c.data_ptr() for c in self.counters) + (st["best_loss"].data_ptr(),)
+        if self._prebook_key != key:
+            if self._best_prev is None:
+                self._best_prev = torch.zeros((), dtype=torch.float32, device=self.device)
+            self._prebook_dev = jet_hip.prebook_struct(self.counters, st["best_loss"], self._best_prev)
+            self._prebook_key = key
+        return self._prebook_dev
 
     def _dp_tail_phase_b(self, loss, grads, terms):
         from .ops import jet_hip
@@ -593,12 +616,14 @@
             self._streams = [torch.cuda.Stream(device=self.flat.device) for _ in (self._ranges or ())]
         return self._ranges
 
-    def run(self, pack=True):
+    def run(self, pack=True, prebook=None):
         prog, fop = self.program, self.program.fused_op
         fs = self.fused_step()
+        if prebook is not None and fs is None:
+            raise RuntimeError("the pre-bookkeeping needs the one-launch fused step")
         if fs is not None:
             J, saved, work = self.buffers()
-            fs.run(saved, J, work, self.flat, pack=pack)
+            fs.run(saved, J, work, self.flat, pack=pack, prebook=prebook)
             return saved, work, 0, fs.tail_kw()
         rng = self.ranges()
         if not rng and not self.persistent:
diff --git a/tensordiffeq_amd/ops/_lib.py b/tensordiffeq_amd/ops/_lib.py
--- a/tensordiffeq_amd/ops/_lib.py
+++ b/tensordiffeq_amd/ops/_lib.py
@@ -8,7 +8,7 @@
 
 _HERE = os.path.dirname(os.path.abspath(__file__))
 LIB_PATH = os.environ.get("TDQ_LIB_PATH") or os.path.join(os.path.dirname(_HERE), "csrc", "libtdq_hip.so")
-ABI_VERSION = 27
+ABI_VERSION = 28
 
 _lock = threading.Lock()
 _lib = None
@@ -37,13 +37,17 @@
         "tdq_jet_bf3_pack": (I, [P, P, I, I, P, I, I, I, P]),
         "tdq_step_tail_bf3": (I, [P, P, P, I, I, P, I, I, I, I, P, I, I, I, P, P, P] + [P, L, P, P, P, P]
                               + [P, I, P, I, P, I, P, I, P]),
+        "tdq_step_tail1_bf3": (I, [P, P, P, I, I, P, I, I, I, I, P, I, I, I, P, P, P] + [P, L, P, P, P, P]
+                               + [P, I, P, I, P, I, P, I, P, P]),
+        "tdq_step_prebook": (I, [P, P]),
+        "tdq_prebook_size": (I, []),
         "tdq_bf3_slab_geometry": (I, [I, I, P, I, I, I, I, P]),
         "tdq_slab_prereduce_bf3": (I, [P, I, I, P, I, I, I, I, I, I, P]),
         "tdq_dp_tail_a_bf3": (I, [P, P, I, I, P, I, I, I, I, P, I, I, I, P, P, P, I, P, I, I, P]),
         "tdq_dp_tail_b_bf3": (I, [P, I, I, P, I, I, I, P, I, P, P, P]),
         "tdq_jet_bf3_scratch_floats": (L, [I, I, P, I, I, I]),
         "tdq_jet_bf3_slab_floats": (L, [I, I, P, I, I]),
-        "tdq_fused_step_launch": (I, [P, P, P, P, I, I, P, I, I, I, P, I, P, P, I, I, I, P]),
+        "tdq_fused_step_launch": (I, [P, P, P, P, I, I, P, I, I, I, P, I, P, P, I, I, I, P, P]),
         "tdq_fused_params_size": (I, []),
         "tdq_jet_fused_lds": (I, [I, P, I, I, I, I]),
         "tdq_device_cus": (I, []),
diff --git a/tensordiffeq_amd/ops/fused_step.py b/tensordiffeq_amd/ops/fused_step.py
--- a/tensordiffeq_amd/ops/fused_step.py
+++ b/tensordiffeq_amd/ops/fused_step.py
@@ -441,7 +441,7 @@
             self.fop2.partials = self.lpart[:self.prow * self.nacc]
             self._side = torch.cuda.Stream(device=dev)
 
-    def run(self, saved, J, work, flat, pack=True):
+    def run(self, saved, J, work, flat, pack=True, prebook=None):
         lib = _lib.load()
         fop, cfg = self.fop, self.cfg
         if pack:
@@ -456,7 +456,8 @@
             rc = lib.tdq_fused_step_launch(self.func, _lib.ptr(self.X), _lib.ptr(scratch), _lib.ptr(work), self.N,
                                            cfg["d_in"], jet_hip._warg(cfg), cfg["d_out"], cfg["n_hidden"], S,
                                            spec_arr, self.G, _lib.ptr(fop.ptrs), _lib.ptr(self.lpart),
-                                           self.prow, self.nacc, int(self.lo), _lib.stream_ptr(flat.device))
+                                           self.prow, self.nacc, int(self.lo), _lib.ptr(prebook),
+                                           _lib.stream_ptr(flat.device))
             _lib.check(rc, "tdq_fused_step_launch")
 
         if side is None:
diff --git a/tensordiffeq_amd/ops/jet_hip.py b/tensordiffeq_amd/ops/jet_hip.py
--- a/tensordiffeq_amd/ops/jet_hip.py
+++ b/tensordiffeq_amd/ops/jet_hip.py
@@ -1,6 +1,7 @@
 from __future__ import annotations
 
 import ctypes
+import os
 
 import torch
 
@@ -192,13 +193,39 @@
     _lib.check(rc, "tdq_slab_prereduce_bf3")
 
 
+class _PreBook(ctypes.Structure):
+    _fields_ = [("c", ctypes.c_void_p * 8), ("n", ctypes.c_int), ("pad", ctypes.c_int),
+                ("best_loss", ctypes.c_void_p), ("best_prev", ctypes.c_void_p)]
+
+
+def prebook_struct(counters, best_loss, best_prev):
+    lib = _lib.load()
+    if len(counters) > 8 or lib.tdq_prebook_size() != ctypes.sizeof(_PreBook):
+        raise ValueError("prebook_struct: more than 8 step counters / FzPreBook layout mismatch")
+    pb = _PreBook()
+    for i, c in enumerate(counters):
+        pb.c[i] = c.data_ptr()
+    pb.n = len(counters)
+    pb.best_loss, pb.best_prev = best_loss.data_ptr(), best_prev.data_ptr()
+    return torch.frombuffer(bytearray(bytes(pb)), dtype=torch.uint8).to(best_loss.device)
+
+
+def step_prebook(pre):
+    _lib.check(_lib.load().tdq_step_prebook(_lib.ptr(pre), _lib.stream_ptr(pre.device)), "tdq_step_prebook")
+
+
+def tail_one_enabled():
+    return os.environ.get("TDQ_TAIL_ONE", "1") != "0"
+
+
 def step_tail(saved, work, grad, fop, book, counters, group_array, n_groups, snapshot, write_images=True,
-              c_first=0, gextra=None, rows=0, lpart=None, n_lblocks=None):
+              c_first=0, gextra=None, rows=0, lpart=None, n_lblocks=None, best_prev=None):
     lib = _lib.load()
     X, P, scratch, cfg, spec, S = saved
     hist = book["hist"]
     carr = (ctypes.c_void_p * max(1, len(counters)))(*[c.data_ptr() for c in counters])
-    rc = lib.tdq_step_tail_bf3(
+    one = best_prev is not None
+    rc = (lib.tdq_step_tail1_bf3 if one else lib.tdq_step_tail_bf3)(
         _lib.ptr(work), _lib.ptr(grad), _lib.ptr(scratch) if write_images else None,
         X.shape[0], cfg["d_in"], _warg(cfg), cfg["d_out"], cfg["n_hidden"], S, *_lo_args(cfg),
         _lib.ptr(fop.partials if lpart is None else lpart), fop.n_blocks if n_lblocks is None else int(n_lblocks),
@@ -208,8 +235,8 @@
         _lib.ptr(book["best_epoch"]), _lib.ptr(book["improved"]), ctypes.cast(carr, ctypes.c_void_p), len(counters),
         ctypes.cast(group_array, ctypes.c_void_p), n_groups,
         _lib.ptr(snapshot) if snapshot is not None else None, int(c_first), _lib.ptr(gextra), int(rows),
-        _lib.stream_ptr(X.device))
-    _lib.check(rc, "tdq_step_tail_bf3")
+        *([_lib.ptr(best_prev)] if one else []), _lib.stream_ptr(X.device))
+    _lib.check(rc, "tdq_step_tail1_bf3" if one else "tdq_step_tail_bf3")
 
 
 class JetMLPFunction(torch.autograd.Function):
```

Result: faster. 378.2 million collocation-pts/s, median of 6 (+1.0%).
